# sunkafei/coffeedb

Hardware: AMD Instinct MI355X
Metric: sa_build_GiB_per_s (higher is better)
Workload: dtype u64

## Files before the change

coffeedb_amd/csrc/capi.hip:

```cpp
#include <dirent.h>

#include <algorithm>
#include <chrono>
#include <condition_variable>
#include <cstdlib>
#include <cstring>
#include <thread>

#include "../../include/coffeedb_gpu.h"
#include "index_impl.h"

using namespace cdb;

namespace {

static_assert((int)Status::Invalid == CDB_E_INVALID && (int)Status::Device == CDB_E_DEVICE && (int)Status::Internal == CDB_E_INTERNAL,
              "errors.h: Status restates the CDB_E_* codes");

void set_error(Index& ix, const std::string& msg) {
    std::lock_guard<std::mutex> g(ix.err_mu);
    ix.err = msg;
}

template <typename F>
// ... 1501 lines not shown
        out->nrows = r.nrows;
        out->nhits = r.nhits;
        out->d_row_ptr = ix.q_rowptr.as<uint64_t>();
        out->d_ids = ix.q_ids.as<int64_t>();
        out->d_counts = ix.q_counts.as<int64_t>();
        if (hits) {
            hits->d_hit_ptr = ix.q_hitptr.as<uint64_t>();
            hits->d_offsets = ix.q_hitoff.as<uint64_t>();
        }
        ix.qstats.query_ms = wall_ms() - t0;
        ix.qstats.nhits = r.nhits;
        ix.qstats.nrows = r.nrows;
    });
}
}

int cdb_query_batch_device(cdb_index* h, const void* d_blob, const uint64_t* d_offsets, uint64_t npat,
                           uint64_t blob_bytes, cdb_device_result* out) {
    (void)blob_bytes;
    return query_batch_device_impl(h, d_blob, d_offsets, npat, out, nullptr);
}

int cdb_query_batch_offsets_device(cdb_index* h, const void* d_blob, const uint64_t* d_offsets, uint64_t npat,
                                   uint64_t blob_bytes, cdb_device_result* out, cdb_device_hits* hits) {
    (void)blob_bytes;
    if (!hits) return CDB_E_INVALID;
    return query_batch_device_impl(h, d_blob, d_offsets, npat, out, hits);
}

uint64_t cdb_size(const cdb_index* h) { return h ? h->ix.size : 0; }
uint64_t cdb_bits(const cdb_index* h) { return h ? h->ix.bits : 0; }
uint64_t cdb_mask(const cdb_index* h) { return h ? h->ix.mask : 0; }
int cdb_sa_width(const cdb_index* h) { return h ? h->ix.width : 0; }

int cdb_sa_copy(cdb_index* h, void* host_out, uint64_t capacity_bytes) {
    if (!h || !host_out) return CDB_E_INVALID;
    return guarded(h, [&] {
        Index& ix = h->ix;
        std::lock_guard<std::mutex> g(ix.mu);
        DeviceScope dscope(ix);
        const uint64_t need = ix.size * (uint64_t)ix.width;
        if (capacity_bytes < need) throw Error("cdb_sa_copy: buffer too small");
        if (need && ix.sa_packed) {
            DevBuf chunk;
            const uint64_t per = std::min<uint64_t>(ix.size, 32ull << 20);
            chunk.alloc(per * 8);
            for (uint64_t first = 0; first < ix.size; first += per) {
                const uint64_t cnt = std::min<uint64_t>(per, ix.size - first);
                sa_expand(ix, first, cnt, chunk.as<uint64_t>());
                CDB_HIP(hipMemcpyAsync(static_cast<char*>(host_out) + first * 8, chunk.p, cnt * 8, hipMemcpyDeviceToHost, ix.stream));
                CDB_HIP(hipStreamSynchronize(ix.stream));
            }
        } else if (need) {
            CDB_HIP(hipMemcpyAsync(host_out, ix.d_sa.p, need, hipMemcpyDeviceToHost, ix.stream));
            CDB_HIP(hipStreamSynchronize(ix.stream));
        }
    });
}

int cdb_set_option(cdb_index* h, const char* name, int64_t value) {
    if (!h || !name) return CDB_E_INVALID;
    Index& ix = h->ix;
    for (const char* o : {"fast_search", "key_directory", "single_query", "search_lanes", "keep_keys", "reference_compat"})
        if (!std::strcmp(name, o)) {
            std::lock_guard<std::mutex> g(ix.mu);
            query_resident_stop(ix);
        }
    if (!std::strcmp(name, "profile")) ix.prof.enabled = value != 0;
    else if (!std::strcmp(name, "reference_compat")) ix.reference_compat = value != 0;
    else if (!std::strcmp(name, "force_doubling")) ix.force_doubling = value != 0;
    else if (!std::strcmp(name, "initial_passes")) ix.initial_passes = (int)value;
    else if (!std::strcmp(name, "sort_variant")) ix.sort_variant = (int)value;
    else if (!std::strcmp(name, "keyhist3")) ix.keyhist3 = value != 0;
    else if (!std::strcmp(name, "key_symbols")) ix.key_symbols = (int)value;
    else if (!std::strcmp(name, "msd_first")) ix.msd_first = value != 0;
    else if (!std::strcmp(name, "msd_pair")) ix.msd_pair = value != 0;
    else if (!std::strcmp(name, "overlap_paircount")) ix.overlap_paircount = value != 0;
    else if (!std::strcmp(name, "key_directory")) { ix.key_directory = value != 0; ix.h_keydir.clear(); ix.keydir_tried = false; }
    else if (!std::strcmp(name, "fuse_records")) ix.fuse_records = value != 0;
    else if (!std::strcmp(name, "sweep_records")) ix.sweep_records = value != 0;
    else if (!std::strcmp(name, "partial_symbol")) ix.partial_symbol = value != 0;
    else if (!std::strcmp(name, "group_sort")) ix.group_sort = value != 0;
    else if (!std::strcmp(name, "list_rounds")) ix.list_rounds = value != 0;
    else if (!std::strcmp(name, "fuse_pairclass")) ix.fuse_pairclass = value != 0;
    else if (!std::strcmp(name, "group_sort_cap")) ix.group_sort_cap = (int)std::max<int64_t>(1, std::min<int64_t>(value, 1 << 20));
    else if (!std::strcmp(name, "vl_keys")) ix.vl_keys = value < 0 ? 0 : (value > 56 ? 56 : (int)value);
    else if (!std::strcmp(name, "pack_sa")) ix.pack_sa = value != 0;
    else if (!std::strcmp(name, "key_cost_model")) ix.key_cost_model = value != 0;
    else if (!std::strcmp(name, "gen_prebased")) ix.gen_prebased = value != 0;
    else if (!std::strcmp(name, "pack_entries")) ix.pack_entries = value != 0;
    else if (!std::strcmp(name, "segmented_sort")) ix.segmented_sort = value != 0;
    else if (!std::strcmp(name, "fold_root")) ix.fold_root = value != 0;
    else if (!std::strcmp(name, "fold_depth1")) ix.fold_depth1 = value != 0;
    else if (!std::strcmp(name, "flags_in_last_pass")) ix.flags_in_last_pass = value != 0;
    else if (!std::strcmp(name, "search_lanes")) ix.search_lanes = (value == 1 || value == 8) ? (int)value : 0;
    else if (!std::strcmp(name, "digit_bits")) ix.digit_bits = (int)value;
    else if (!std::strcmp(name, "fuse_keygen")) ix.fuse_keygen = value != 0;
    else if (!std::strcmp(name, "force_big_path")) ix.force_big_path = value != 0;
    else if (!std::strcmp(name, "debug_fail_build")) ix.debug_fail_build = value != 0;
    else if (!std::strcmp(name, "debug_append_path")) ix.debug_append_path = value == 1 || value == 2 ? (int)value : 0;
    else if (!std::strcmp(name, "debug_no_segcap")) ix.debug_no_segcap = value != 0;
    else if (!std::strcmp(name, "debug_starve_group")) ix.debug_starve_group = (int)value;
    else if (!std::strcmp(name, "self_check")) ix.self_check = value < 0 ? 0 : value > 3 ? 3 : (int)value;
    else if (!std::strcmp(name, "premap_generation")) ix.premap_generation = value != 0;
    else if (!std::strcmp(name, "proof_cancel")) {
        if (value) proof_stop(ix);
    }
    else if (!std::strcmp(name, "debug_damage_after_build")) ix.debug_damage_after_build = value < 0 ? 0 : (uint64_t)value;
    else if (!std::strcmp(name, "debug_fail_self_check")) ix.debug_fail_self_check = value != 0;
    else if (!std::strcmp(name, "plain_tile_order")) ix.rws.plain_order = value != 0;
    else if (!std::strcmp(name, "key_coding")) ix.key_coding = (int)value;
    else if (!std::strcmp(name, "narrow_keys")) ix.narrow_keys = value != 0;
    else if (!std::strcmp(name, "single_query")) ix.use_single_query = value != 0;
    else if (!std::strcmp(name, "resident_query")) {
        std::lock_guard<std::mutex> g(ix.mu);
        if (value != 1) query_resident_stop(ix);
        ix.resident_mode = value <= 0 ? 0 : value == 1 ? 1 : 2;
        ix.resident_query = ix.resident_mode == 1;
        ix.single_streak = 0;
    }
    else if (!std::strcmp(name, "bucket_group_limit")) ix.bucket_group_limit = (uint64_t)value;
    else if (!std::strcmp(name, "query_hit_budget"))
        ix.query_hit_budget = value > 0 ? std::min<uint64_t>((uint64_t)value, 1ull << 31) : 1;
    else if (!std::strcmp(name, "coalesce_queries")) ix.coalesce_queries = value != 0;
    else if (!std::strcmp(name, "fast_search")) ix.use_fast_search = value != 0;
    else if (!std::strcmp(name, "wave_rows")) ix.use_wave_rows = value != 0;
    else if (!std::strcmp(name, "keep_keys")) ix.keep_keys = value != 0;
    else {
        set_error(ix, std::string("unknown option: ") + name);
        return CDB_E_INVALID;
    }
    return CDB_OK;
}

int cdb_get_stat(const cdb_index* h, const char* name, double* value) {
    if (!h || !name || !value) return CDB_E_INVALID;
    const BuildStats& b = h->ix.bstats;
    const QueryStats& q = h->ix.qstats;
    struct { const char* n; double v; } tab[] = {
        {"build_ms", b.build_ms}, {"alloc_ms", b.alloc_ms}, {"free_ms", b.free_ms}, {"rounds", (double)b.rounds}, {"ext_rounds", (double)b.ext_rounds},
        {"dbl_rounds", (double)b.dbl_rounds}, {"unresolved_after_initial", (double)b.unresolved_initial},
        {"unresolved_max", (double)b.unresolved_max}, {"sort_passes", (double)b.sort_passes},
        {"sort_passes_skipped", (double)b.sort_passes_skipped}, {"isa_built", (double)b.isa_built}, {"fused_keygen", (double)b.fused_keygen}, {"dense_keys", (double)b.dense_keys}, {"key_layout", (double)b.key_layout}, {"bucketed", (double)b.bucketed}, {"bucket_groups", (double)b.bucket_groups}, {"segmented", (double)b.segmented}, {"fused_records", (double)b.fused_records}, {"sweep_records", (double)b.sweep_records}, {"vl_key_bits", (double)b.vl_key_bits}, {"partial_levels", (double)b.partial_levels}, {"list_rounds", (double)b.list_rounds}, {"pairclass_fused", (double)b.pairclass_fused}, {"group_sorts", (double)b.group_sorts}, {"group_sort_fallbacks", (double)b.group_sort_fallbacks}, {"vl_avg_len", b.vl_avg_len}, {"vl_rate", b.vl_rate}, {"vl_est_unresolved", b.vl_est_unresolved}, {"fixed_est_unresolved", b.fixed_est_unresolved}, {"gen_prebased", (double)b.gen_prebased}, {"root_folded", (double)b.root_folded}, {"flags_in_last_pass", (double)b.flags_in_last_pass}, {"msd_first", (double)b.msd_first}, {"bucket_low_digits", (double)b.bucket_low_digits}, {"key_directory_cells", h->ix.h_keydir.empty() ? 0.0 : (double)(h->ix.h_keydir.size() - 1)}, {"group_fallbacks", (double)h->ix.group_fallbacks}, {"dense_key_retries", (double)h->ix.dense_key_retries}, {"self_check_fallbacks", (double)h->ix.self_check_fallbacks}, {"sa_packed", h->ix.sa_packed ? 1.0 : 0.0}, {"sa_bytes_per_entry", h->ix.sa_packed ? 5.0 : (double)h->ix.width}, {"self_check_pairs", (double)h->ix.self_check_pairs}, {"self_check_ms", h->ix.self_check_ms}, {"self_check_coverage", h->ix.size > 1 ? (double)h->ix.self_check_pairs / (double)(h->ix.size - 1) : 0.0},
        {"order_proved", (h->ix.proof.state.load() == 2 || h->ix.proof.state.load() == 3 || (h->ix.self_check == 2 && h->ix.width != 0)) ? 1.0 : 0.0},
        {"proof_state", (double)h->ix.proof.state.load()}, {"proof_ms", h->ix.proof.ms}, {"proof_repair_ms", h->ix.proof.repair_ms},
        {"proof_pairs", (double)h->ix.proof.pairs}, {"proof_bad_pairs", (double)h->ix.proof.found[0]}, {"proof_invalid_entries", (double)h->ix.proof.found[1]}, {"proof_skipped_pairs", (double)h->ix.proof.skipped}, {"proof_mixed_pairs", (double)h->ix.proof.mixed},
        {"proof_runs", (double)h->ix.proof.runs}, {"pool_big_mallocs", (double)DevPool::get().big_mallocs()}, {"premap_ms", h->ix.proof.premap_ms}, {"premap_bytes", (double)h->ix.proof.premap_bytes},
        {"key_symbols", (double)b.key_symbols}, {"symbol_bits", (double)b.symbol_bits},
        {"alphabet", (double)b.alphabet}, {"digit_bits", (double)b.digit_bits}, {"final_depth", (double)b.final_depth}, {"compat_rotations", (double)b.compat_rotations},
        {"compat_depth", (double)b.compat_depth},
        {"host_upload_ms", h->ix.host_upload_ms}, {"host_free_ms", h->ix.host_free_ms},
        {"resident_answers", (double)h->ix.res_answers}, {"launched_answers", (double)h->ix.launched_answers}, {"resident_mode", (double)h->ix.resident_mode},
        {"cluster_table_bytes", h->ix.clu.valid ? (double)(h->ix.clu.bytes() + h->ix.idt.bytes()) : 0.0}, {"cluster_classes", (double)h->ix.clu.nclasses},
        {"cluster_prepare_ms", h->ix.clu.prepare_ms}, {"cluster_ms", h->ix.clu.last_ms}, {"cluster_resorted", h->ix.clu.resorted ? 1.0 : 0.0},
        {"removes", (double)h->ix.rm.calls}, {"remove_compactions", (double)h->ix.rm.compactions}, {"remove_rebuilds", (double)h->ix.rm.rebuilds},
        {"remove_docs", (double)h->ix.rm.docs}, {"remove_bytes", (double)h->ix.rm.bytes}, {"remove_ms", h->ix.rm.last_ms},
        {"appends", (double)h->ix.ap.calls}, {"append_merges", (double)h->ix.ap.merges}, {"append_rebuilds", (double)h->ix.ap.rebuilds},
        {"append_docs", (double)h->ix.ap.docs}, {"append_bytes", (double)h->ix.ap.bytes}, {"append_ms", h->ix.ap.last_ms},
        {"append_keys_kept", (double)h->ix.ap.with_keys},
        {"render_ms", h->ix.rnd.last_ms}, {"render_page_bytes", (double)h->ix.rnd.page_bytes}, {"render_spans", (double)h->ix.rnd.spans},
        {"query_ms", q.query_ms}, {"query_upload_ms", q.upload_ms}, {"query_device_ms", q.device_ms}, {"query_download_ms", q.download_ms}, {"query_hits", (double)q.nhits}, {"query_rows", (double)q.nrows},
        {"query_batches", (double)q.batches}, {"query_spec_batches", (double)q.spec_batches}, {"query_spec_spills", (double)q.spec_spills},
        {"query_wave_batches", (double)q.wave_batches}, {"query_sort_batches", (double)q.sort_batches}, {"query_sort_chunks", (double)q.sort_chunks},
        {"query_empty_batches", (double)q.empty_batches},
    };
    for (auto& e : tab)
        if (!std::strcmp(e.n, name)) {
            *value = e.v;
            return CDB_OK;
        }
    return CDB_E_INVALID;
}

int cdb_profile_get(cdb_index* h, const char* kernel, double* total_ms, uint64_t* launches, uint64_t* bytes) {
    if (!h || !kernel) return CDB_E_INVALID;
    std::lock_guard<std::mutex> g(h->ix.mu);
    auto it = h->ix.prof.recs.find(kernel);
    if (it == h->ix.prof.recs.end()) return CDB_E_INVALID;
    if (total_ms) *total_ms = it->second.ms;
    if (launches) *launches = it->second.launches;
    if (bytes) *bytes = it->second.bytes;
    return CDB_OK;
}

int cdb_profile_dump(cdb_index* h, char* buf, size_t cap) {
    if (!h || !buf || cap == 0) return CDB_E_INVALID;
    std::lock_guard<std::mutex> g(h->ix.mu);
    std::string s;
    for (auto& kv : h->ix.prof.recs) {
        char line[256];
        std::snprintf(line, sizeof(line), "%s %.6f %llu %llu\n", kv.first.c_str(), kv.second.ms,
                      (unsigned long long)kv.second.launches, (unsigned long long)kv.second.bytes);
        s += line;
    }
    std::strncpy(buf, s.c_str(), cap - 1);
    buf[cap - 1] = 0;
    return CDB_OK;
}

int cdb_debug_verify(cdb_index* h, uint64_t out[5]) {
    if (!h || !out) return CDB_E_INVALID;
    return guarded(h, [&] {
        Index& ix = h->ix;
        std::lock_guard<std::mutex> g(ix.mu);
        DeviceScope dscope(ix);
        if (ix.width == 0) throw Error("index has not been built");
        verify_suffix_array(ix, out);
    });
}

int cdb_debug_self_check(cdb_index* h, int full, uint64_t out[2]) {
    if (!h || !out) return CDB_E_INVALID;
    return guarded(h, [&] {
        Index& ix = h->ix;
        std::lock_guard<std::mutex> g(ix.mu);
        DeviceScope dscope(ix);
        if (ix.width == 0) throw Error("index has not been built");
        spot_check_suffix_array(ix, full ? 0u : (uint32_t)std::min<uint64_t>(1u << 15, ix.size > 1 ? ix.size - 1 : 1), out);
    });
}

int cdb_proof_wait(cdb_index* h, double timeout_ms) {
    if (!h) return CDB_E_INVALID;
    const double t0 = wall_ms();
    for (;;) {
        const int st = h->ix.proof.state.load();
// ... 94 lines not shown
```

coffeedb_amd/csrc/index_impl.h:

```cpp
#pragma once
#include <atomic>
#include <condition_variable>
#include <functional>
#include <mutex>
#include <thread>
#include <string>
#include <vector>

#include "../../include/coffeedb_gpu.h"
#include "common.h"
#include "radix_sort.h"

namespace cdb {

constexpr int TEXT_PAD = 128;

struct BuildStats {
    double build_ms = 0, alloc_ms = 0, free_ms = 0;
    int rounds = 0;
    int ext_rounds = 0;
    int dbl_rounds = 0;
    uint64_t unresolved_initial = 0;
    uint64_t unresolved_max = 0;
    int sort_passes = 0;
    int sort_passes_skipped = 0;
    int isa_built = 0;
    int fused_keygen = 0;
    int key_layout = 0;
    int dense_keys = 0;
    int bucketed = 0;
    int bucket_low_digits = 0;
    int bucket_groups = 0;
    int root_folded = 0;
    int flags_in_last_pass = 0;
    int msd_first = 0;
    int gen_prebased = 0;
    int fused_records = 0;
    int sweep_records = 0;
    int pairclass_fused = 0;
    int list_rounds = 0;
    int group_sorts = 0, group_sort_fallbacks = 0;
    int partial_levels = 0;
    int vl_key_bits = 0;
    double vl_avg_len = 0, vl_rate = 0, vl_est_unresolved = 0, fixed_est_unresolved = 0;
    int segmented = 0;
    uint64_t gather_items = 0;
    int key_symbols = 0, symbol_bits = 0, alphabet = 0, digit_bits = 8;
    uint64_t final_depth = 0;
    uint64_t compat_rotations = 0, compat_depth = 0;
};

struct QueryStats {
    double query_ms = 0;
    double upload_ms = 0, device_ms = 0, download_ms = 0;
    uint64_t nhits = 0, nrows = 0;
    uint64_t batches = 0;
    uint64_t spec_batches = 0, spec_spills = 0;
    uint64_t wave_batches = 0;
    uint64_t sort_batches = 0, sort_chunks = 0;
    uint64_t empty_batches = 0;
};

struct KeptKeys {
    uint64_t* k64 = nullptr;
    uint32_t* k32 = nullptr;
    uint8_t* low = nullptr;
    int low_bits = 0, low_bytes = 0;
    __host__ __device__ __forceinline__ bool present() const { return k64 != nullptr || k32 != nullptr; }
    __device__ __forceinline__ uint64_t low_at(uint64_t i) const {
        return low_bytes == 2 ? (uint64_t)reinterpret_cast<const uint16_t*>(low)[i] : (uint64_t)low[i];
    }
    __device__ __forceinline__ uint64_t at(uint64_t i) const {
        if (k64) return k64[i];
        const uint64_t h = k32[i];
        if (!low_bits) return h;
        return (h << low_bits) | low_at(i);
    }
    __device__ __forceinline__ int cmp_range(uint64_t i, uint64_t klo, uint64_t khi) const {
        uint64_t key;
        if (k64) {
            key = k64[i];
        } else {
            const uint64_t h = k32[i];
            if (low) {
                const uint64_t a = klo >> low_bits, b = khi >> low_bits;
                if (h < a) return -1;
                if (h > b) return 1;
                if (h > a && h < b) return 0;
                key = (h << low_bits) | low_at(i);
            } else {
                key = h;
            }
        }
        return key < klo ? -1 : (key > khi ? 1 : 0);
    }
    __device__ __forceinline__ void put(uint64_t i, uint64_t key) const {
        if (k64) k64[i] = key;
        if (k32) k32[i] = (uint32_t)(key >> low_bits);
        if (low) {
            const uint64_t l = key & ((1ull << low_bits) - 1ull);
            if (low_bytes == 2) reinterpret_cast<uint16_t*>(low)[i] = (uint16_t)l;
            else low[i] = (uint8_t)l;
        }
    }
    __device__ __forceinline__ void copy(const KeptKeys& src, uint64_t from, uint64_t to) const {
        if (k64) k64[to] = src.k64[from];
        if (k32) k32[to] = src.k32[from];
        if (low) {
            if (low_bytes == 2) reinterpret_cast<uint16_t*>(low)[to] = reinterpret_cast<const uint16_t*>(src.low)[from];
            else low[to] = src.low[from];
        }
    }
    uint64_t bytes_per_slot() const { return (k64 ? 8 : 0) + (k32 ? 4 : 0) + (low ? low_bytes : 0); }
};
struct SingleKeys {
    KeptKeys keys;
    int nsym = 0;
    bool decisive = false;
    uint64_t klo = 0, khi = 0;
    bool ranged = false;
    uint64_t lo0 = 0, hi0 = 0;
};

struct Sa40 {
// ... 54 lines not shown
    bool overlap_paircount = true;
    bool res_running = false;
    uint32_t res_seq = 0;
    SingleKeys res_keys;
    bool use_fast_search = true;

    std::vector<int64_t> ids;
    std::vector<uint64_t> doc_start{0};
    std::string host_text;
    bool host_tables_valid = true;
    bool host_text_valid = true;

    uint64_t bits = 1, mask = 1, size = 0;
    int off_bits = 1;
    int width = 0;
    uint64_t ndocs = 0;

    DevBuf d_text_owned;
    const uint8_t* d_text = nullptr;
    bool text_padded = false;
    DevBuf d_doc_start;
    DevBuf d_ids;
    DevBuf d_sa;
    DevBuf d_sa_hi;
    bool sa_packed = false;
    bool gen_prebased = true;
    TileBaseWorkspace tbw;
    bool key_cost_model = true;
    bool pack_sa = true;
    void release_sa() {
        d_sa.release();
        d_sa_hi.release();
        sa_packed = false;
        clu.drop();
        idt.drop();
    }
    template <typename T> typename SaOf<T>::ptr sa_view() const;
    bool sa_sorted = false;
    DevBuf d_keys;
    DevBuf d_symmap_q;
    uint16_t h_symmap_q[256] = {};
    DevBuf d_keys32, d_keylow;
    int key_low_bits = 0;
    int key_low_bytes = 0;
    int key_nsym = 0;
    uint32_t key_base = 0;
    void drop_keys() {
        d_keys.release();
        d_keys32.release();
        d_keylow.release();
        key_nsym = 0;
        key_low_bits = 0;
        key_low_bytes = 0;
        h_keydir.clear();
        h_keydir.shrink_to_fit();
        keydir_tried = false;
    }
    std::vector<uint32_t> h_keydir;
    int keydir_shift = 0, keydir_bits = 0;
    bool keydir_tried = false;
    bool key_directory = true;
    DevBuf d_pivots;
    int pivot_levels = 0;

    RadixWorkspace rws;
    MsdWorkspace msd_ws;
    DevBuf scan_partials;
    uint64_t q_spec_cap = 0;
    DevBuf q_spec;
    DevBuf q_pat, q_offs, q_left, q_right, q_hoff, q_keys0, q_keys1, q_flags, q_rowptr, q_ids, q_counts, q_hitptr, q_hitoff;

    bool reference_compat = true;
    bool force_doubling = false;
    int initial_passes = 0;
    int key_symbols = 0;
    int sort_variant = 0;
    int search_lanes = 0;
    bool flags_in_last_pass = true;
    bool fold_depth1 = true;
    bool fold_root = true;
    bool segmented_sort = true;
    bool fuse_records = true;
    bool fuse_pairclass = true;
    bool list_rounds = true;
    int group_sort_cap = 4096;
    bool group_sort = true;
    bool partial_symbol = true;
    int vl_keys = 2;
    bool vl_off_once = false;
    bool sweep_records = true;
    bool pack_entries = true;
    bool msd_first = true;
    bool msd_pair = true;
    bool keyhist3 = true;
    int dense_key_retries = 0;
    int group_fallbacks = 0;
    uint64_t bucket_group_limit = 0;
    uint64_t self_check_pairs = 0;
    double self_check_ms = 0;
    int self_check = 3;
    int self_check_fallbacks = 0;
    bool debug_fail_self_check = false;
    struct Proof {
        std::thread th;
        std::atomic<int> state{0};
        std::atomic<bool> cancel{false};
        hipStream_t stream = nullptr;
        void* d_out = nullptr;
        double ms = 0, repair_ms = 0;
        uint64_t pairs = 0;
        uint64_t found[2] = {0, 0};
        uint64_t skipped = 0;
        uint64_t mixed = 0;
        uint64_t runs = 0;
        bool of_loaded_file = false;
        std::atomic<bool> busy{false};
        bool want_proof = false;
        double premap_ms = 0;
        uint64_t premap_bytes = 0;
    } proof;
    bool premap_generation = false;
    bool proof_in_repair = false;
    uint64_t debug_damage_after_build = 0;
    bool debug_no_segcap = false;
    int debug_starve_group = 0;
    bool debug_fail_build = false;
    bool force_big_path = false;
    bool fuse_keygen = true;
    int digit_bits = 0;
    bool narrow_keys = true;
    int key_coding = 0;
    uint64_t query_hit_budget = 1ull << 31;

    struct ClusterTables {
        bool valid = false;
        uint64_t nclasses = 0;
        bool resorted = false;
        DevBuf class_of_doc;
        DevBuf class_rep;
        double prepare_ms = 0, last_ms = 0;
        uint64_t bytes() const { return class_of_doc.bytes + class_rep.bytes; }
        void drop() {
            valid = false;
            nclasses = 0;
            class_of_doc.release();
            class_rep.release();
        }
    } clu;
    struct IdTable {
        bool valid = false;
        bool ids_ascend = true;
        DevBuf id_sorted, id_doc;
        uint64_t bytes() const { return id_sorted.bytes + id_doc.bytes; }
        void drop() {
            valid = false;
            ids_ascend = true;
            id_sorted.release();
            id_doc.release();
        }
    } idt;
    struct RenderStats {
        double last_ms = 0;
        uint64_t page_bytes = 0, spans = 0;
    } rnd;

    struct RemoveStats {
// ... 227 lines not shown
```

coffeedb_amd/csrc/radix_sort.h:

```cpp
#pragma once
#include <cstdlib>

#include "common.h"

namespace cdb {

constexpr int RS_MAX_PASSES = 16;

constexpr uint64_t RS_VAL_MASK = (1ull << 54) - 1;
constexpr uint32_t RS_SPIN_LIMIT_GROUPED = 1u << 18;
constexpr uint32_t RS_SPIN_LIMIT_PLAIN = 1u << 22;
constexpr int RS_GROUP = 8;

struct NoVal {};

template <typename K>
__global__ __launch_bounds__(256) void rs_hist_kernel(const K* __restrict__ keys, uint64_t n, int begin_bit,
                                                      int npass, int dbits, uint32_t last_mask,
                                                      unsigned long long* __restrict__ ghist) {
    __shared__ uint32_t sh[RS_MAX_PASSES * 256];
    for (int i = threadIdx.x; i < npass * 256; i += 256) sh[i] = 0;
    __syncthreads();
    const uint64_t stride = (uint64_t)gridDim.x * 256;
    for (uint64_t i = (uint64_t)blockIdx.x * 256 + threadIdx.x; i < n; i += stride) {
// ... 108 lines not shown
    int rec_low_bits = 0;
    uint32_t part_m = 1, part_r = 0, part_s = 0;
    bool msd_pair = false;
    uint32_t pair_span = 0, pair_r = 0, pair_s = 0;
    const uint64_t* tile_doc = nullptr;
    const unsigned long long* tile_base = nullptr;
    uint8_t* vout_hi = nullptr;
};
struct TextGenPair : TextGen {};
struct TextGenRec : TextGen {};
constexpr int RS_GEN_LOOK = 64;
#ifndef RS_GEN_ABL
#define RS_GEN_ABL 0
#endif
#ifndef RS_SEG_ABL
#define RS_SEG_ABL 0
#endif



struct RsDiv24 { uint32_t mul, sh; };
inline RsDiv24 rs_div24_make(uint32_t d) {
    uint32_t L = 0;
    while ((1ull << L) < d) ++L;
    const uint64_t m = ((1ull << (24 + L)) + d - 1) / d;
    return RsDiv24{(uint32_t)(m << 7), L + 7};
}
__device__ __forceinline__ uint32_t rs_div24(uint32_t x, uint32_t mul, uint32_t sh) { return __umulhi(x << 8, mul) >> sh; }

template <typename G>
inline bool rs_pair_setup(G& gen, uint32_t base, uint32_t span) {
    const uint64_t b2 = (uint64_t)base * base;
    if (base < 2 || base > 255 || span == 0 || span >= (1u << 24) || b2 >= (1u << 24)) return false;
    if ((uint64_t)span * b2 >= (1u << 24)) return false;
    if ((uint64_t)span * b2 * b2 > (1ull << 32)) return false;
    for (uint32_t sh = 0; sh < 32; ++sh) {
        const uint64_t r = ((1ull << sh) + span - 1) / span;
        if (r >= (1u << 24) || (b2 - 1) * r >= (1ull << 32)) break;
        bool ok = true;
        for (uint64_t a = 0; a < b2 && ok; ++a) ok = ((a * r) >> sh) == a / span;
        if (ok) {
            gen.pair_span = span;
            gen.pair_r = (uint32_t)r;
            gen.pair_s = sh;
            return true;
        }
    }
    return false;
}

struct NoSeg {};
struct SegInfo {
    unsigned long long begin, end;
    uint32_t tile_begin, top;
    unsigned long long rot_a, rot_b;
};
__device__ __forceinline__ unsigned long long rs_seg_rotated(const SegInfo& si, unsigned long long slot) {
    if (si.rot_b == 0) return slot;
    const unsigned long long r = slot - si.begin, len = si.end - si.begin;
    if (r < si.rot_a) return slot;
    return r < si.rot_b ? slot + (len - si.rot_b) : slot - (si.rot_b - si.rot_a);
}
struct SegArgs {
    const uint32_t* tile_seg = nullptr;
    const SegInfo* segs = nullptr;
    uint32_t tiles = 0;
    uint32_t start_stride = 0;
};
struct SegEdge {
    unsigned long long first, last;
    unsigned long long pos;
    uint32_t cnt, pad;
};
struct SegFinalArgs : SegArgs {
    uint64_t* eout = nullptr;
    uint32_t* elo = nullptr;
    uint8_t* ehi = nullptr;
    uint8_t* flags = nullptr;
    SegEdge* edges = nullptr;
    int hi_shift = 0;
    int low_bits = 0;
    uint32_t kbase = 2;
    unsigned long long kmagic = 0;
};

struct SegFinalKeepArgs : SegArgs {
    uint8_t* flags = nullptr;
    SegEdge* edges = nullptr;
    int low_bits = 0;
    uint32_t kbase = 2;
    unsigned long long kmagic = 0;
    unsigned long long* tile_sums = nullptr;
    uint32_t sums_tile = 1;
    unsigned long long msd_m = 0;
};

struct SegFinalKeepMsdArgs : SegFinalKeepArgs {};

__device__ __forceinline__ uint64_t rs_pack_key(const uint32_t* __restrict__ s_words, uint32_t li, int nsym, uint32_t base,
                                                uint32_t rem) {
    const uint32_t wi = li >> 2, sel = li & 3u;
    const uint32_t b2 = base * base, b3 = b2 * base;
    const uint32_t pw[5] = {1u, base, b2, b3, b3 * base};
    uint64_t kk = 0;
    uint32_t lo = s_words[wi];
#pragma unroll
    for (int w = 0; w < 4; ++w) {
        const int q = 4 * w;
        if (q >= nsym) break;
        const int r = nsym - q < 4 ? nsym - q : 4;
        const uint32_t hi = s_words[wi + w + 1];
        uint32_t x = __builtin_amdgcn_alignbyte(hi, lo, sel);
        lo = hi;
        if (rem < (uint32_t)(q + 4)) x = rem <= (uint32_t)q ? 0u : (x & ((1u << (8u * (rem - (uint32_t)q))) - 1u));
        uint32_t v = x & 0xFFu;
        if (r > 1) v = v * base + ((x >> 8) & 0xFFu);
        if (r > 2) v = v * base + ((x >> 16) & 0xFFu);
        if (r > 3) v = v * base + (x >> 24);
        kk = (r == 4 && pw[4] == 0u) ? ((kk << 32) | v) : kk * pw[r] + v;
    }
    return kk;
}

__device__ __forceinline__ uint64_t rs_doc_upper(const uint64_t* __restrict__ doc_start, uint64_t lo, uint64_t hi,
                                                 uint64_t p) {
    while (lo < hi) {
        const uint64_t mid = lo + (hi - lo + 1) / 2;
        if (doc_start[mid] <= p) lo = mid; else hi = mid - 1;
    }
    return lo;
}

static __global__ __launch_bounds__(256) void rs_tiledoc_kernel(const uint64_t* __restrict__ doc_start, uint64_t ndocs,
                                                                uint64_t n, uint64_t tile_elems, uint64_t tiles,
                                                                uint64_t* __restrict__ tile_doc) {
    const uint64_t t = (uint64_t)blockIdx.x * 256 + threadIdx.x;
    if (t > tiles) return;
    const uint64_t p = t * tile_elems < n ? t * tile_elems : n - 1;
    tile_doc[t] = rs_doc_upper(doc_start, 0, ndocs - 1, p);
}

template <typename K, typename V, typename Cfg, typename Gen = NoGen, typename W = NoVal, typename Seg = NoSeg>
__global__ __launch_bounds__(Cfg::NT, Cfg::MINW) void rs_onesweep_kernel(
    const K* __restrict__ kin, K* __restrict__ kout, const V* __restrict__ vin, V* __restrict__ vout, uint64_t n,
    int shift, uint32_t dmask, const unsigned long long* __restrict__ digit_start, uint64_t* __restrict__ status,
    uint32_t* __restrict__ ticket, uint32_t epoch, uint32_t* __restrict__ err, Gen gen = Gen(),
    const W* __restrict__ win = nullptr, W* __restrict__ wout = nullptr, int aux_shift = -1, Seg seg = Seg()) {
    constexpr bool GEN = !std::is_same<Gen, NoGen>::value;
    constexpr bool SEG = !std::is_same<Seg, NoSeg>::value;
    constexpr bool FINAL = std::is_same<Seg, SegFinalArgs>::value;
    constexpr bool KEEPM = std::is_same<Seg, SegFinalKeepMsdArgs>::value;
    constexpr bool KEEP = std::is_same<Seg, SegFinalKeepArgs>::value || KEEPM;
    constexpr bool FLAGS = FINAL || KEEP;
    static_assert(!SEG || (!GEN && !Cfg::DMA), "segmented passes: materialised records");
    static_assert(!FLAGS || Cfg::REUSE || KEEPM, "flag-writing passes: shared staging (the MSD-first last pass also runs with keys and values staged at once)");
    constexpr bool HAS_V = !std::is_same<V, NoVal>::value;
    constexpr bool HAS_W = !std::is_same<W, NoVal>::value;
    using WS = typename std::conditional<HAS_W, W, uint8_t>::type;
    static_assert(!HAS_W || KEEPM || (Cfg::REUSE && HAS_V && !Cfg::DMA), "the auxiliary byte needs the shared-staging configuration");
    constexpr int IPT = Cfg::IPT;
    constexpr bool REUSE = Cfg::REUSE && HAS_V;
    constexpr bool EARLYV = (Cfg::EARLYV || REUSE) && HAS_V;
    constexpr int NT = Cfg::NT;
    constexpr int NW = NT / 64;
    constexpr bool NTM = Cfg::NONTEMP;
    constexpr int TILE = NT * IPT;
// ... 611 lines not shown
            if (real) {
                const uint64_t lmask = (1ull << seg.low_bits) - 1ull;
                const uint32_t a = tstart, b = tstart + (uint32_t)real - 1u;
                if constexpr (KEEPM) {
                    e.first = ktop + (uint64_t)s_keys[a];
                    e.last = ktop + (uint64_t)s_keys[b];
                } else {
                    e.first = ((uint64_t)s_keys[a] << seg.low_bits) | ((uint64_t)s_aux[HAS_W ? a : 0] & lmask);
                    e.last = ((uint64_t)s_keys[b] << seg.low_bits) | ((uint64_t)s_aux[HAS_W ? b : 0] & lmask);
                }
            }
            seg.edges[tile * 256 + d] = e;
        }
    }

    if constexpr (!REUSE) {
#pragma unroll
        for (int j = 0; j < IPT; ++j) {
            const uint32_t i = j * NT + tid;
            if (i < valid) {
                const K k = s_keys[i];
                const uint32_t dd = (uint32_t)(k >> shift) & dmask;
                const uint64_t dst = s_gbase[dd] + i;
                if constexpr (KEEPM) {
                    bool head = true, tail = true;
                    if (i > 0) head = s_keys[i - 1] != k;
                    if (i + 1 < valid) tail = s_keys[i + 1] != k;
                    const uint64_t kf = ktop + (uint64_t)k;
                    uint32_t f = head ? 1u : 0u;
                    if (!(head && tail)) {
                        const bool exhausted = seg.kmagic ? (kf - __umul64hi(kf, seg.kmagic) * seg.kbase) == 0
                                                          : (kf & (uint64_t)(seg.kbase - 1u)) == 0;
                        if (!exhausted) f |= 2u;
                    }
                    seg.flags[dst] = (uint8_t)f;
                    if ((f & 2u) && seg.tile_sums) {
                        atomicAdd(seg.tile_sums + 2 * (dst / seg.sums_tile), 1ull);
                        if (f & 1u) atomicAdd(seg.tile_sums + 2 * (dst / seg.sums_tile) + 1, 1ull);
                    }
                    rs_store<NTM>(kout + dst, (K)(kf >> 8));
                    if constexpr (HAS_W) rs_store<NTM>(wout + dst, (W)(kf & 0xFFu));
                    rs_store<NTM>(vout + dst, (V)s_vals[i]);
                    continue;
                }
                if (!GEN || kout) rs_store<NTM>(kout + dst, k);
                if constexpr (HAS_V) rs_store<NTM>(vout + dst, (V)s_vals[i]);
            }
        }
    } else {
        uint8_t dig[IPT];
#pragma unroll
        for (int j = 0; j < IPT; ++j) {
            const uint32_t i = j * NT + tid;
            dig[j] = 0;
            if (i < valid) {
                const K k = s_keys[i];
                uint32_t dd;
                if constexpr (KEEPM) dd = (uint32_t)(k >> shift) & dmask;
                else dd = digit_of(k, s_aux[HAS_W ? i : 0]);
                if constexpr (recs) dd = (uint32_t)s_gen[i];
                dig[j] = (uint8_t)dd;
                if constexpr (FLAGS) {
                    const uint32_t lmask = seg.low_bits >= 32 ? 0xFFFFFFFFu : (1u << seg.low_bits) - 1u;
                    uint32_t ac = 0;
                    if constexpr (!KEEPM) ac = (uint32_t)s_aux[HAS_W ? i : 0] & lmask;
                    bool head = true, tail = true;
                    bool cmp = true;
                    if constexpr (FINAL) cmp = !(RS_SEG_ABL & 4);
                    if constexpr (KEEPM) {
                        if (i > 0) head = s_keys[i - 1] != k;
                        if (i + 1 < valid) tail = s_keys[i + 1] != k;
                    } else if (cmp) {
                        if (i > 0) head = s_keys[i - 1] != k || ((uint32_t)s_aux[HAS_W ? i - 1 : 0] & lmask) != ac;
                        if (i + 1 < valid) tail = s_keys[i + 1] != k || ((uint32_t)s_aux[HAS_W ? i + 1 : 0] & lmask) != ac;
                    }
                    uint32_t f = head ? 1u : 0u;
                    if (!(head && tail)) {
                        const uint64_t kc = KEEPM ? ktop + (uint64_t)k : (((uint64_t)k << seg.low_bits) | (uint64_t)ac);
                        const bool exhausted = seg.kmagic ? (kc - __umul64hi(kc, seg.kmagic) * seg.kbase) == 0
                                                          : (kc & (uint64_t)(seg.kbase - 1u)) == 0;
                        if (!exhausted) f |= 2u;
                    }
                    if constexpr (FINAL) {
                        if (!(RS_SEG_ABL & 1)) seg.flags[rs_seg_rotated(si, s_gbase[dd] + i)] = (uint8_t)f;
                        continue;
                    } else {
                        const uint64_t slot = s_gbase[dd] + i;
                        seg.flags[slot] = (uint8_t)f;
                        if ((f & 2u) && seg.tile_sums) {
                            atomicAdd(seg.tile_sums + 2 * (slot / seg.sums_tile), 1ull);
                            if (f & 1u) atomicAdd(seg.tile_sums + 2 * (slot / seg.sums_tile) + 1, 1ull);
                        }
                    }
                }
                if constexpr (KEEPM) {
                    const uint64_t kf = ktop + (uint64_t)k;
                    rs_store<NTM>(kout + s_gbase[dd] + i, (K)(kf >> 8));
                    if constexpr (HAS_W) rs_store<NTM>(wout + s_gbase[dd] + i, (W)(kf & 0xFFu));
                    continue;
                }
                if (!GEN || kout) rs_store<NTM>(kout + s_gbase[dd] + i, k);
                if constexpr (HAS_W && !W32G) {
                    if (!GEN || wout) rs_store<NTM>(wout + s_gbase[dd] + i, (W)s_aux[i]);
                }
            }
        }
        __syncthreads();
        if constexpr (W32G) {
#pragma unroll
            for (int j = 0; j < IPT; ++j) s_vals[rank[j]] = (VS)aux[j];
            __syncthreads();
#pragma unroll
            for (int j = 0; j < IPT; ++j) {
                const uint32_t i = j * NT + tid;
                if (i < valid) rs_store<NTM>(wout + s_gbase[dig[j]] + i, (W)s_vals[i]);
            }
            __syncthreads();
        }
#pragma unroll
        for (int j = 0; j < IPT; ++j) s_vals[rank[j]] = val[j];
        __syncthreads();
#pragma unroll
        for (int j = 0; j < IPT; ++j) {
            const uint32_t i = j * NT + tid;
            if constexpr (FINAL) {
                if (i < valid && !(RS_SEG_ABL & 2)) {
                    const unsigned long long slot = rs_seg_rotated(si, s_gbase[dig[j]] + i);
                    const uint32_t hi32 = (uint32_t)s_aux[HAS_W ? i : 0] >> seg.hi_shift;
                    if (seg.elo) {
                        seg.elo[slot] = (uint32_t)s_vals[i];
                        seg.ehi[slot] = (uint8_t)hi32;
                    } else {
                        seg.eout[slot] = ((uint64_t)hi32 << 32) | (uint64_t)s_vals[i];
                    }
                }
            } else {
                if constexpr (GEN && sizeof(VS) == 8) {
                    if (gen.vout_hi) {
                        if (i < valid) {
                            const uint64_t dst = s_gbase[dig[j]] + i;
                            const uint64_t e = (uint64_t)s_vals[i];
                            reinterpret_cast<uint32_t*>(vout)[dst] = (uint32_t)e;
                            gen.vout_hi[dst] = (uint8_t)(e >> 32);
                        }
                        continue;
                    }
                }
                if (i < valid) rs_store<NTM>(vout + s_gbase[dig[j]] + i, (V)s_vals[i]);
            }
        }
    }
}

static __global__ __launch_bounds__(256) void rs_seg_edge_fix_kernel(const SegEdge* __restrict__ edges, const uint32_t* __restrict__ tile_seg,
                                                                     const SegInfo* __restrict__ segs, uint32_t tiles,
                                                                     uint8_t* __restrict__ flags, uint32_t kbase, unsigned long long kmagic,
                                                                     unsigned long long* __restrict__ tile_sums = nullptr,
                                                                     uint32_t sums_tile = 1, const uint32_t* __restrict__ err = nullptr) {
    const uint32_t t = blockIdx.x, d = threadIdx.x;
    if (t >= tiles) return;
    if (err && *err) return;
    const SegEdge e = edges[(size_t)t * 256 + d];
    if (!e.cnt) return;
    const SegInfo si = segs[tile_seg ? tile_seg[t] : 0u];
    const uint32_t t0 = si.tile_begin;
    if (t == t0) return;
    uint32_t lo = t0, hi = t;
    if (edges[(size_t)(t - 1) * 256 + d].pos < e.pos) {
        lo = t - 1;
    } else {
        if (edges[(size_t)t0 * 256 + d].pos >= e.pos) return;
        hi = t - 1;
        while (hi - lo > 1) {
            const uint32_t mid = lo + (hi - lo) / 2;
            if (edges[(size_t)mid * 256 + d].pos < e.pos) lo = mid; else hi = mid;
        }
    }
    const SegEdge pe = edges[(size_t)lo * 256 + d];
    if (pe.last != e.first) return;
    const bool exhausted = kmagic ? (e.first - __umul64hi(e.first, kmagic) * kbase) == 0 : (e.first & (uint64_t)(kbase - 1u)) == 0;
    auto change = [&](unsigned long long slot, uint32_t clear, uint32_t set) {
        const uintptr_t a = reinterpret_cast<uintptr_t>(flags + slot);
        unsigned int* w = reinterpret_cast<unsigned int*>(a & ~(uintptr_t)3);
        const uint32_t sh = 8u * (uint32_t)(a & 3u);
        uint32_t before, after;
        if (clear) {
            before = (atomicAnd(w, ~(clear << sh)) >> sh) & 0xFFu;
            after = before & ~clear;
        } else {
            before = (atomicOr(w, set << sh) >> sh) & 0xFFu;
            after = before | set;
        }
        if (tile_sums && before != after) {
            const long long da = (long long)((after >> 1) & 1u) - (long long)((before >> 1) & 1u);
            const long long db = (long long)((after >> 1) & after & 1u) - (long long)((before >> 1) & before & 1u);
            unsigned long long* ts = tile_sums + 2 * (slot / sums_tile);
            if (da) atomicAdd(ts, (unsigned long long)da);
            if (db) atomicAdd(ts + 1, (unsigned long long)db);
        }
    };
    const unsigned long long sb = rs_seg_rotated(si, e.pos), sa_ = rs_seg_rotated(si, e.pos - 1);
    change(sb, 1u, 0u);
    if (!exhausted) {
        change(sb, 0u, 2u);
        change(sa_, 0u, 2u);
    }
}

static __global__ __launch_bounds__(256) void rs_lane_order_probe_kernel(uint32_t* __restrict__ bad) {
    __shared__ uint32_t cnt[4][256];
    __shared__ uint32_t ref[4][256];
// ... 861 lines not shown
```

coffeedb_amd/csrc/records_sweep.h:

```cpp
#pragma once
#include "radix_sort.h"

namespace cdb {

#ifndef RS_SWEEP_ABL
#define RS_SWEEP_ABL 0
#endif
#ifndef RS_SWEEP_UNALIGNED
#define RS_SWEEP_UNALIGNED 0
#endif
__device__ __forceinline__ int rs_uniform(int x) {
    int y = __builtin_amdgcn_readfirstlane(x);
    asm volatile("" : "+s"(y));
    return y;
}
__device__ __forceinline__ uint32_t rs_wave_incl_scan(uint32_t x) {
    uint32_t v = x;
    v += (uint32_t)__builtin_amdgcn_update_dpp(0, (int)x, 0x111, 0xf, 0xf, false);
    v += (uint32_t)__builtin_amdgcn_update_dpp(0, (int)x, 0x112, 0xf, 0xf, false);
    v += (uint32_t)__builtin_amdgcn_update_dpp(0, (int)x, 0x113, 0xf, 0xf, false);
    v += (uint32_t)__builtin_amdgcn_update_dpp(0, (int)v, 0x114, 0xf, 0xe, false);
    v += (uint32_t)__builtin_amdgcn_update_dpp(0, (int)v, 0x118, 0xf, 0xc, false);
    v += (uint32_t)__builtin_amdgcn_update_dpp(0, (int)v, 0x142, 0xa, 0xf, false);
    v += (uint32_t)__builtin_amdgcn_update_dpp(0, (int)v, 0x143, 0xc, 0xf, false);
    return v;
}

constexpr int RS_SWEEP_TILE = RS_GEN8_TILE;
constexpr uint32_t RS_SWEEP_DOCS = 768;

template <typename W>
__global__ __launch_bounds__(512, 8) void rs_sweep_records_kernel(TextGen gen, const uint16_t* __restrict__ codeslot, uint64_t n, uint32_t tiles,
                                                                  uint32_t g0, uint32_t g1, uint64_t gstart, uint32_t* __restrict__ kout,
                                                                  uint32_t* __restrict__ vout, W* __restrict__ wout) {
    constexpr int NT = 512, IPT = 16, TILE = RS_SWEEP_TILE, NW = NT / 64;
    static_assert(NT * IPT == TILE, "tile shape");
    constexpr int abl = RS_SWEEP_ABL;
    constexpr uint32_t TEXTB = ((TILE + RS_GEN_LOOK + 15) / 16) * 16;
    constexpr uint32_t NBLK = TILE / 32, DOCS = 184;
    __shared__ __attribute__((aligned(16))) uint8_t s_text[TEXTB];
    __shared__ uint16_t s_cs[256];
    __shared__ __attribute__((aligned(16))) uint32_t s_doc[4 * DOCS];
    __shared__ uint8_t s_slotc[256];
    __shared__ uint32_t s_whist[NW][256];
    __shared__ __attribute__((aligned(8))) uint32_t s_blk[2 * (NBLK + 1)];
    __shared__ uint64_t s_gbase[256];
    __shared__ uint32_t s_wsum[8];
    __shared__ uint32_t s_flag;
    __shared__ __attribute__((aligned(16))) uint16_t s_idx[TILE];
    uint8_t* const s_dig = reinterpret_cast<uint8_t*>(s_idx);

    const int tid = threadIdx.x, lane = tid & 63, wave = tid >> 6;
    const uint32_t x = blockIdx.x & 7u, slot = blockIdx.x >> 3;
    const uint64_t tile = (uint64_t)((slot / RS_GROUP) * 8u + x) * RS_GROUP + slot % RS_GROUP;
    if (tile >= (uint64_t)tiles) return;
    const uint64_t base = tile * TILE;
    const uint32_t valid = (uint32_t)((n - base) < (uint64_t)TILE ? (n - base) : (uint64_t)TILE);

    const uint64_t ga = base + (uint64_t)tid * 16, gb = base + (uint64_t)TILE + (uint64_t)tid * 16;
    const bool has_b = (uint32_t)tid * 16 < TEXTB - (uint32_t)TILE;
    const bool oka = gen.padded ? (ga < n + RS_GEN_LOOK) : (ga + 16 <= n);
    const bool okb = has_b && (gen.padded ? (gb < n + RS_GEN_LOOK) : (gb + 16 <= n));
    uint4 ta = make_uint4(0, 0, 0, 0), tb = make_uint4(0, 0, 0, 0);
    if (oka) ta = *reinterpret_cast<const uint4*>(gen.text + ga);
    if (okb) tb = *reinterpret_cast<const uint4*>(gen.text + gb);
    uint64_t my_base = 0;
    if ((uint32_t)tid >= g0 && (uint32_t)tid < g1) my_base = (uint64_t)gen.tile_base[tile * 256 + (uint64_t)tid];
    if (tid < 256) {
        const uint32_t e = codeslot[tid];
        s_cs[tid] = (uint16_t)(((e >> 8) >= g0 && (e >> 8) < g1) ? e : (e | 0xFF00u));
        s_slotc[tid] = gen.slotmap[tid];
    }
    const uint64_t dlo = gen.tile_doc[tile], dhi = gen.tile_doc[tile + 1];
    for (int i = tid; i < NW * 256; i += NT) (&s_whist[0][0])[i] = 0;
    if ((uint32_t)tid <= NBLK) s_blk[2 * tid] = 0;
    if (tid == 0) s_flag = 0;
    const uint32_t ndl = (uint32_t)(dhi - dlo);
    const bool docs_in_lds = dhi - dlo + 2 <= (uint64_t)DOCS;
    uint64_t dreg0 = 0;
    if (docs_in_lds && (uint32_t)tid < ndl + 2) dreg0 = gen.doc_start[dlo + tid];
    __syncthreads();
    if (docs_in_lds && (uint32_t)tid < ndl + 2) {
        const uint32_t d = (uint32_t)tid;
        const int64_t diff = (int64_t)(dreg0 - base);
// ... 124 lines not shown
        const uint32_t l1 = li + 1u, wi = l1 >> 2, sel = l1 & 3u;
        const uint32_t w0 = s_words[wi], w1 = s_words[wi + 1], w2 = s_words[wi + 2];
        uint32_t x0 = __builtin_amdgcn_alignbyte(w1, w0, sel);
        uint32_t x1 = __builtin_amdgcn_alignbyte(w2, w1, sel);
        uint32_t x2 = 0;
        if (nsx > 8) x2 = __builtin_amdgcn_alignbyte(s_words[wi + 3], w2, sel);
        if (__builtin_expect(__builtin_amdgcn_readfirstlane((int)(__builtin_amdgcn_ballot_w64(rem1 < (uint32_t)nsx) != 0)) != 0, 0)) {
            if (rem1 < (uint32_t)nsx) {
                x0 = rem1 >= 4u ? x0 : (rem1 == 0u ? 0u : (x0 & ((1u << (8u * rem1)) - 1u)));
                x1 = rem1 >= 8u ? x1 : (rem1 <= 4u ? 0u : (x1 & ((1u << (8u * (rem1 - 4u))) - 1u)));
                x2 = rem1 >= 12u ? x2 : (rem1 <= 8u ? 0u : (x2 & ((1u << (8u * (rem1 - 8u))) - 1u)));
            }
        }
        uint64_t acc = 0;
#pragma unroll
        for (int q = 0; q < 5; ++q) {
            if (2 * q < ns1) {
                const uint32_t xw = q < 2 ? x0 : (q < 4 ? x1 : x2);
                uint32_t pv, mult;
                if (2 * q + 1 < ns1) {
                    pv = __builtin_amdgcn_udot4(xw, (q & 1) ? whi : wlo, 0u, false);
                    mult = B2;
                } else {
                    pv = (q & 1) ? ((xw >> 16) & 0xFFu) : (xw & 0xFFu);
                    mult = B;
                }
                if (q == 0) acc = pv;
                else if (q == 1) acc = (uint64_t)(uint32_t)acc * mult + pv;
                else acc = acc * (uint64_t)mult + pv;
            }
        }
        if (part_on) {
            const uint32_t xq = ns1 < 4 ? x0 : (ns1 < 8 ? x1 : x2);
            const uint32_t cq = (xq >> (8 * (ns1 & 3))) & 0xFFu;
            acc = acc * (uint64_t)gen.part_m + (uint64_t)((cq * gen.part_r) >> gen.part_s);
        }
        const uint64_t dst = s_gbase[sl] + (uint64_t)p;
        if (abl & 8) {
            if (acc == 0x123456789ull && e64 == 77) kout[dst] = 1;
            return;
        }
        kout[dst] = (uint32_t)(acc >> gen.rec_low_bits);
        vout[dst] = (uint32_t)e64;
        wout[dst] = (W)((acc & lmask) | ((e64 >> 32) << gen.rec_low_bits));
    };
    if (docs_in_lds && s_flag == 0 && valid == (uint32_t)TILE && !(abl & 4)) {
        const int bits = gen.bits;
        auto rec = [&](uint32_t p) {
            const uint32_t li = s_idx[p];
            const uint2 bk = *reinterpret_cast<const uint2*>(&s_blk[2 * (li >> 5)]);
            const uint32_t doff = bk.y + 16u * (uint32_t)__builtin_popcount(bk.x & ~(0xFFFFFFFEu << (li & 31u)));
            const uint4 dc = *reinterpret_cast<const uint4*>(reinterpret_cast<const uint8_t*>(s_doc) + doff);
            emit(p, li, (((uint64_t)dc.y << 32) | dc.x) + ((uint64_t)li << bits), (uint32_t)((int32_t)dc.z - (int32_t)li - 1));
        };
        if (kept == (uint32_t)TILE) {
            for (uint32_t p = tid; p < (uint32_t)TILE; p += 2 * NT) {
                rec(p);
                rec(p + NT);
            }
        } else {
            for (uint32_t p = tid; p < kept; p += NT) rec(p);
        }
    } else {
        for (uint32_t p = tid; p < kept; p += NT) {
            const uint32_t li = s_idx[p];
            const uint64_t pos = base + li;
            uint64_t dd = dlo, ds = 0, de = 1ull << 40;
            if (!(abl & 4)) {
                dd = rs_doc_upper(gen.doc_start, dlo, dhi, pos);
                ds = gen.doc_start[dd];
                de = gen.doc_start[dd + 1];
            }
            const uint64_t left = de - pos - 1ull;
            emit(p, li, ((pos - ds) << gen.bits) + dd, left < 64ull ? (uint32_t)left : 64u);
        }
    }
}

struct VlTables {
    const uint16_t* sym = nullptr;
    const uint16_t* dec = nullptr;
    int key_bits = 0;
    int end_len = 0;
};
constexpr uint32_t RS_VL_BITW = ((RS_GEN8_TILE + RS_GEN_LOOK) * 7 + 31) / 32 + 4;

template <typename W>
__global__ __launch_bounds__(512, 6) void rs_sweep_records_vl_kernel(TextGen gen, const uint16_t* __restrict__ codeslot, VlTables vl, uint64_t n,
                                                                     uint32_t tiles, uint32_t g0, uint32_t g1, uint64_t gstart,
                                                                     uint32_t* __restrict__ kout, uint32_t* __restrict__ vout, W* __restrict__ wout) {
    constexpr int NT = 512, IPT = 16, TILE = RS_SWEEP_TILE, NW = NT / 64;
    constexpr uint32_t LOOK = RS_GEN_LOOK, NBLK = TILE / 32, DOCS = 256, SL = 128;
    static_assert(LOOK == 64, "four staging threads cover the look-ahead");
    __shared__ uint32_t s_bits[RS_VL_BITW];
    __shared__ __attribute__((aligned(16))) uint16_t s_boff[TILE + LOOK + 8];
    __shared__ __attribute__((aligned(16))) uint16_t s_idx[TILE];
    __shared__ uint32_t s_whist[NW][SL];
    __shared__ uint16_t s_cs[256];
    __shared__ uint16_t s_vl[SL];
    __shared__ uint16_t s_dec[128];
    __shared__ __attribute__((aligned(16))) uint32_t s_doc[4 * DOCS + 4];
    __shared__ __attribute__((aligned(8))) uint32_t s_blk[2 * (NBLK + 1)];
    __shared__ uint64_t s_gbase[SL];
    __shared__ uint32_t s_wsum[16];
    __shared__ uint32_t s_flag;
    uint8_t* const s_dig = reinterpret_cast<uint8_t*>(s_idx);

    const int tid = threadIdx.x, lane = tid & 63, wave = tid >> 6;
    const uint32_t x = blockIdx.x & 7u, slot = blockIdx.x >> 3;
    const uint64_t tile = (uint64_t)((slot / RS_GROUP) * 8u + x) * RS_GROUP + slot % RS_GROUP;
    if (tile >= (uint64_t)tiles) return;
    const uint64_t base = tile * TILE;
    const uint32_t valid = (uint32_t)((n - base) < (uint64_t)TILE ? (n - base) : (uint64_t)TILE);

    const uint64_t ga = base + (uint64_t)tid * 16, gb = base + (uint64_t)TILE + (uint64_t)tid * 16;
    const bool has_b = (uint32_t)tid * 16 < LOOK;
    const bool oka = gen.padded ? (ga < n + LOOK) : (ga + 16 <= n);
    const bool okb = has_b && (gen.padded ? (gb < n + LOOK) : (gb + 16 <= n));
    uint4 ta = make_uint4(0, 0, 0, 0), tb = make_uint4(0, 0, 0, 0);
    if (oka) ta = *reinterpret_cast<const uint4*>(gen.text + ga);
    if (okb) tb = *reinterpret_cast<const uint4*>(gen.text + gb);
    uint64_t my_base = 0;
    if ((uint32_t)tid >= g0 && (uint32_t)tid < g1) my_base = (uint64_t)gen.tile_base[tile * 256 + (uint64_t)tid];
    if (tid < 256) {
        const uint32_t e = codeslot[tid];
        s_cs[tid] = (uint16_t)(((e >> 8) >= g0 && (e >> 8) < g1) ? e : (e | 0xFF00u));
    }
    if (tid < (int)SL) {
        s_vl[tid] = vl.sym[tid];
        s_dec[tid] = vl.dec[tid];
    }
    const uint64_t dlo = gen.tile_doc[tile], dhi = gen.tile_doc[tile + 1];
    for (int i = tid; i < NW * (int)SL; i += NT) (&s_whist[0][0])[i] = 0;
    for (uint32_t i = tid; i < RS_VL_BITW; i += NT) s_bits[i] = 0;
    if ((uint32_t)tid <= NBLK) s_blk[2 * tid] = 0;
    if (tid == 0) s_flag = 0;
    const uint32_t ndl = (uint32_t)(dhi - dlo);
    const bool docs_in_lds = dhi - dlo + 2 <= (uint64_t)DOCS;
    uint64_t dreg0 = 0;
    if (docs_in_lds && (uint32_t)tid < ndl + 2) dreg0 = gen.doc_start[dlo + tid];
    __syncthreads();
    if (docs_in_lds && (uint32_t)tid < ndl + 2) {
        const uint32_t d = (uint32_t)tid;
        const int64_t diff = (int64_t)(dreg0 - base);
        const int32_t rel = diff < -(1ll << 30) ? -(1 << 30) : (diff > (1ll << 30) ? (1 << 30) : (int32_t)diff);
        const uint64_t eb = ((base - dreg0) << gen.bits) + dlo + d;
        s_doc[4 * d] = (uint32_t)eb;
        s_doc[4 * d + 1] = (uint32_t)(eb >> 32);
        if (d >= 1) s_doc[4 * d - 2] = (uint32_t)rel;
        if (d >= 1 && rel <= (int32_t)TILE) {
            const uint32_t bit = 1u << ((uint32_t)rel & 31u);
            if (atomicOr(&s_blk[2 * ((uint32_t)rel >> 5)], bit) & bit) s_flag = 1;
        }
    }
    auto fetch = [&](uint64_t g, bool ok, uint4 w, uint32_t* c) {
        c[0] = w.x; c[1] = w.y; c[2] = w.z; c[3] = w.w;
        if (!ok) {
#pragma unroll
            for (int q = 0; q < 4; ++q) {
                c[q] = 0;
#pragma unroll
                for (int b = 0; b < 4; ++b) c[q] |= (uint32_t)((g + 4 * q + b < n) ? gen.text[g + 4 * q + b] : (uint8_t)0) << (8 * b);
            }
        }
    };
    auto pack4 = [&](const uint32_t* v, uint32_t& word, uint32_t& wlen, uint32_t& lens4) {
// ... 60 lines not shown
                o += (lens[k >> 3] >> (4 * (k & 7))) & 0xFu;
            }
            *reinterpret_cast<uint4*>(&s_boff[pos0]) = make_uint4(packed[0], packed[1], packed[2], packed[3]);
            *reinterpret_cast<uint4*>(&s_boff[pos0 + 8]) = make_uint4(packed[4], packed[5], packed[6], packed[7]);
            uint32_t bo = at;
#pragma unroll
            for (int h = 0; h < 2; ++h) {
                const uint32_t wi = bo >> 5, sh = bo & 31u;
                const uint32_t xh = (uint32_t)(piece[h] >> 32), xl = (uint32_t)piece[h];
                atomicOr(&s_bits[wi], __builtin_amdgcn_alignbit(0u, xh, sh));
                atomicOr(&s_bits[wi + 1], __builtin_amdgcn_alignbit(xh, xl, sh));
                atomicOr(&s_bits[wi + 2], __builtin_amdgcn_alignbit(xl, 0u, sh));
                bo += plen[h];
            }
            return o;
        };
        (void)emit_bits(wpre + inclA - totA, pieceA, plenA, lensA, (uint32_t)tid * 16);
        if (has_b) {
            const uint32_t end = emit_bits(all + inclB - totB, pieceB, plenB, lensB, (uint32_t)TILE + (uint32_t)tid * 16);
            if ((uint32_t)tid * 16 + 16 == LOOK) s_boff[TILE + LOOK] = (uint16_t)end;
        }
    }
    __syncthreads();
    constexpr int WCHUNK = IPT * 64;
    const uint32_t wbase = wave * WCHUNK + lane;
    uint32_t info[IPT];
    {
        uint32_t sl[IPT];
#pragma unroll
        for (int j = 0; j < IPT; ++j) sl[j] = s_dig[wbase + j * 64];
#pragma unroll
        for (int j = 0; j < IPT; ++j) {
            uint32_t inf = 0xFFu << 16;
            if (sl[j] != 0xFFu) inf = atomicAdd(&s_whist[wave][sl[j]], 1u) | (sl[j] << 16);
            info[j] = inf;
        }
    }
    __syncthreads();
    uint32_t wc[NW], cnt = 0, incl = 0;
    if (tid < (int)SL) {
#pragma unroll
        for (int w = 0; w < NW; ++w) {
            wc[w] = s_whist[w][tid];
            cnt += wc[w];
        }
        incl = cnt;
    } else if (tid >= 256) {
        incl = cnt = (uint32_t)__builtin_popcount(s_blk[2 * (tid - 256)]);
    }
    incl = rs_wave_incl_scan(incl);
    if (lane == 63) s_wsum[8 + wave] = incl;
    __syncthreads();
    const uint32_t kept = s_wsum[8] + s_wsum[9];
    {
        uint32_t wpre = 0;
        if (tid < (int)SL) {
            if (wave == 1) wpre = s_wsum[8];
            const uint32_t excl = wpre + incl - cnt;
            uint32_t run = excl;
#pragma unroll
            for (int w = 0; w < NW; ++w) {
                s_whist[w][tid] = run;
                run += wc[w];
            }
            s_gbase[tid] = my_base - gstart - (uint64_t)excl;
        } else if (tid >= 256) {
#pragma unroll
            for (int w = 4; w < NW; ++w)
                if (w < wave) wpre += s_wsum[8 + w];
            const uint32_t excl = wpre + incl - cnt;
            s_blk[2 * (tid - 256) + 1] = excl * 16u;
            if (tid == 511) s_blk[2 * NBLK + 1] = (excl + cnt) * 16u;
        }
    }
    __syncthreads();
#pragma unroll
    for (int k = 0; k < IPT; ++k) {
        const uint32_t sl = info[k] >> 16;
        if (sl != 0xFFu) s_idx[s_whist[wave][sl] + (info[k] & 0xFFFFu)] = (uint16_t)(wbase + k * 64);
    }
    __syncthreads();

    const int KB1 = vl.key_bits - 1;
    const uint64_t lmask = (1ull << gen.rec_low_bits) - 1ull;
    auto emit = [&](uint32_t p, uint32_t li, uint64_t e64, uint32_t endbit) {
        const uint32_t o0 = s_boff[li];
        const uint32_t wi = o0 >> 5, sh = o0 & 31u;
        const uint32_t w0 = s_bits[wi], w1 = s_bits[wi + 1], w2 = s_bits[wi + 2];
        const uint32_t hi = __builtin_amdgcn_alignbit(w0, w1, 32u - sh), lo = __builtin_amdgcn_alignbit(w1, w2, 32u - sh);
        const uint64_t top = sh ? (((uint64_t)hi << 32) | lo) : (((uint64_t)w0 << 32) | w1);
        const uint32_t dv = s_dec[(uint32_t)(top >> 57)];
        const uint32_t sl = dv & 0xFFu, len = dv >> 8;
        const uint32_t avail = endbit - (o0 + len);
        const uint32_t take = avail < (uint32_t)KB1 ? avail : (uint32_t)KB1;
        uint64_t kb = (top << len) >> (64 - KB1);
        kb &= ~0ull << ((uint32_t)KB1 - take);
        const uint64_t key = (kb << 1) | (uint64_t)(avail + (uint32_t)vl.end_len > (uint32_t)KB1 ? 1u : 0u);
        const uint64_t dst = s_gbase[sl] + (uint64_t)p;
        kout[dst] = (uint32_t)(key >> gen.rec_low_bits);
        vout[dst] = (uint32_t)e64;
        wout[dst] = (W)((key & lmask) | ((e64 >> 32) << gen.rec_low_bits));
    };
    if (docs_in_lds && s_flag == 0 && valid == (uint32_t)TILE) {
        const int bits = gen.bits;
        for (uint32_t p = tid; p < kept; p += NT) {
            const uint32_t li = s_idx[p];
            const uint2 bk = *reinterpret_cast<const uint2*>(&s_blk[2 * (li >> 5)]);
            const uint32_t doff = bk.y + 16u * (uint32_t)__builtin_popcount(bk.x & ~(0xFFFFFFFEu << (li & 31u)));
            const uint4 dc = *reinterpret_cast<const uint4*>(reinterpret_cast<const uint8_t*>(s_doc) + doff);
            const int32_t rn = (int32_t)dc.z;
            const uint32_t relend = rn < (int32_t)(TILE + LOOK) ? (uint32_t)rn : (uint32_t)(TILE + LOOK);
            emit(p, li, (((uint64_t)dc.y << 32) | dc.x) + ((uint64_t)li << bits), (uint32_t)s_boff[relend]);
        }
    } else {
        for (uint32_t p = tid; p < kept; p += NT) {
            const uint32_t li = s_idx[p];
            const uint64_t pos = base + li;
            const uint64_t dd = rs_doc_upper(gen.doc_start, dlo, dhi, pos);
            const uint64_t ds = gen.doc_start[dd], de = gen.doc_start[dd + 1];
            const uint64_t rel = de - base;
            const uint32_t relend = rel < (uint64_t)(TILE + LOOK) ? (uint32_t)rel : (uint32_t)(TILE + LOOK);
            emit(p, li, ((pos - ds) << gen.bits) + dd, (uint32_t)s_boff[relend]);
        }
    }
}

__global__ __launch_bounds__(512, 8) void rs_sweep_msd_kernel(TextGen gen, uint64_t n, uint32_t tiles, uint32_t* __restrict__ kout,
                                                              uint32_t* __restrict__ vout) {
    constexpr int NT = 512, IPT = 16, TILE = RS_SWEEP_TILE, NW = NT / 64;
    constexpr uint32_t TEXTB = ((TILE + RS_GEN_LOOK + 15) / 16) * 16;
    constexpr uint32_t DOCS = 384;
    constexpr uint32_t NBLK = TILE / 32;
    __shared__ __attribute__((aligned(16))) uint8_t s_text[TEXTB];
    __shared__ uint8_t s_code[256];
    __shared__ __attribute__((aligned(8))) uint32_t s_doc[2 * DOCS + 2];
    __shared__ uint32_t s_whist[NW][256];
    __shared__ __attribute__((aligned(8))) uint32_t s_blk[2 * (NBLK + 1)];
    __shared__ uint32_t s_gbase[256];
    __shared__ uint32_t s_wsum[8];
    __shared__ uint32_t s_flag;
    __shared__ __attribute__((aligned(16))) uint16_t s_idx[TILE];
    uint8_t* const s_dig = reinterpret_cast<uint8_t*>(s_idx);

    const int tid = threadIdx.x, lane = tid & 63, wave = tid >> 6;
    const uint32_t x = blockIdx.x & 7u, slot = blockIdx.x >> 3;
    const uint64_t tile = (uint64_t)((slot / RS_GROUP) * 8u + x) * RS_GROUP + slot % RS_GROUP;
    if (tile >= (uint64_t)tiles) return;
    const uint64_t base = tile * TILE;
    const uint32_t valid = (uint32_t)((n - base) < (uint64_t)TILE ? (n - base) : (uint64_t)TILE);

    const uint64_t ga = base + (uint64_t)tid * 16, gb = base + (uint64_t)TILE + (uint64_t)tid * 16;
    const bool has_b = (uint32_t)tid * 16 < TEXTB - (uint32_t)TILE;
    const bool oka = gen.padded ? (ga < n + RS_GEN_LOOK) : (ga + 16 <= n);
    const bool okb = has_b && (gen.padded ? (gb < n + RS_GEN_LOOK) : (gb + 16 <= n));
    uint4 ta = make_uint4(0, 0, 0, 0), tb = make_uint4(0, 0, 0, 0);
    if (oka) ta = *reinterpret_cast<const uint4*>(gen.text + ga);
    if (okb) tb = *reinterpret_cast<const uint4*>(gen.text + gb);
    uint32_t tnext = 0;
    if (lane == 63 && ga + 16 < n) tnext = (uint32_t)gen.text[ga + 16];
    uint64_t my_base = 0;
    if (tid < 256) {
        my_base = (uint64_t)gen.tile_base[tile * 256 + (uint64_t)tid];
        s_code[tid] = (uint8_t)gen.symmap[tid];
    }
    const uint64_t dlo = gen.tile_doc[tile], dhi = gen.tile_doc[tile + 1];
    for (int i = tid; i < NW * 256; i += NT) (&s_whist[0][0])[i] = 0;
    if ((uint32_t)tid <= NBLK) s_blk[2 * tid] = 0;
    if (tid == 0) s_flag = 0;
    const uint32_t ndl = (uint32_t)(dhi - dlo);
    const bool docs_in_lds = dhi - dlo + 2 <= (uint64_t)DOCS;
    uint64_t dreg0 = 0, dreg1 = 0;
    if (docs_in_lds) {
        if ((uint32_t)tid < ndl + 2) dreg0 = gen.doc_start[dlo + tid];
        if ((uint32_t)tid + NT < ndl + 2) dreg1 = gen.doc_start[dlo + tid + NT];
    }
    __syncthreads();
    if (docs_in_lds) {
        auto put = [&](uint32_t d, uint64_t ds) {
            const int64_t diff = (int64_t)(ds - base);
            const int32_t rel = diff < -(1ll << 30) ? -(1 << 30) : (diff > (1ll << 30) ? (1 << 30) : (int32_t)diff);
            s_doc[2 * d] = (uint32_t)(((base - ds) << gen.bits) + dlo + d);
            if (d >= 1) s_doc[2 * d - 1] = (uint32_t)rel;
            if (d >= 1 && rel <= (int32_t)TILE) {
                const uint32_t bit = 1u << ((uint32_t)rel & 31u);
// ... 155 lines not shown
        vout[dst] = ent;
    };
    if (docs_in_lds && s_flag == 0 && valid == (uint32_t)TILE) {
        constexpr int U = 2;
        const int bits = gen.bits;
#pragma nounroll
        for (uint32_t p0 = tid; p0 < (uint32_t)TILE; p0 += U * NT) {
            uint32_t li[U];
            uint2 bk[U], dc[U];
#pragma unroll
            for (int u = 0; u < U; ++u) li[u] = s_idx[p0 + u * NT];
#pragma unroll
            for (int u = 0; u < U; ++u) bk[u] = *reinterpret_cast<const uint2*>(&s_blk[2 * (li[u] >> 5)]);
#pragma unroll
            for (int u = 0; u < U; ++u) {
                const uint32_t doff = bk[u].y + 8u * (uint32_t)__builtin_popcount(bk[u].x & ~(0xFFFFFFFEu << (li[u] & 31u)));
                dc[u] = *reinterpret_cast<const uint2*>(reinterpret_cast<const uint8_t*>(s_doc) + doff);
            }
#pragma unroll
            for (int u = 0; u < U; ++u) emit(p0 + u * NT, li[u], dc[u].x + (li[u] << bits), dc[u].y - li[u]);
        }
    } else {
        for (uint32_t p = tid; p < valid; p += NT) {
            const uint32_t li = s_idx[p];
            const uint64_t pos = base + li;
            const uint64_t dd = rs_doc_upper(gen.doc_start, dlo, dhi, pos);
            const uint64_t ds = gen.doc_start[dd], de = gen.doc_start[dd + 1];
            const uint64_t left = de - pos;
            emit(p, li, (uint32_t)(((pos - ds) << gen.bits) + dd), left < 64ull ? (uint32_t)left : 64u);
        }
    }
}

inline bool rs_sweep_records_ok(uint32_t base, int nsym) { return base <= 255u && nsym >= 2 && nsym - 1 <= 10; }
template <typename G>
inline bool rs_part_setup(G& gen, uint32_t base, uint32_t m) {
    gen.part_m = 1;
    gen.part_r = gen.part_s = 0;
    if (m < 2 || base < 2 || base > 256) return false;
    for (uint32_t sh = 0; sh < 24; ++sh) {
        const uint64_t r = (((uint64_t)m << sh) + base - 1) / base;
        if (r >= (1u << 24)) break;
        bool ok = true;
        for (uint64_t c = 0; c < base && ok; ++c) ok = ((c * r) >> sh) == c * m / base;
        if (ok) {
            gen.part_m = m;
            gen.part_r = (uint32_t)r;
            gen.part_s = sh;
            return true;
        }
    }
    return false;
}

template <typename W>
void radix_sweep_records(hipStream_t s, Profiler& prof, uint32_t* k, uint32_t* v, W* w, uint64_t n, const TextGen& gen_in, const uint16_t* d_codeslot,
                         uint32_t g0, uint32_t g1,
                         uint64_t gstart, uint64_t gelems, const uint32_t* d_tile_seg, const SegInfo* d_segs, uint32_t nseg, uint32_t seg_tiles,
                         int lead, int npass, unsigned long long* d_hist_out, SortStats* stats) {
    if (!gen_in.tile_base || !gen_in.tile_doc || !d_codeslot || !gen_in.slotmap) throw InternalError("radix_sweep_records: tile bases / documents / slots missing (internal)");
    if (!rs_sweep_records_ok(gen_in.base, gen_in.nsym)) throw InternalError("radix_sweep_records: key shape (internal)");
    const uint32_t tiles8 = (uint32_t)ceil_div(n, (uint64_t)RS_SWEEP_TILE);
    const uint32_t grid = (uint32_t)(ceil_div(tiles8, 8u * RS_GROUP) * 8u * RS_GROUP);
    CDB_HIP(hipMemsetAsync(d_hist_out, 0, (size_t)nseg * 8 * 256 * sizeof(uint64_t), s));
    int t = prof.begin(s);
    hipLaunchKernelGGL((rs_sweep_records_kernel<W>), dim3(grid), dim3(512), 0, s, gen_in, d_codeslot, n, tiles8, g0, g1, gstart, k, v, w);
    prof.end(t, (std::string("rs_sweep_records") + (sizeof(W) == 1 ? "_w8" : (sizeof(W) == 2 ? "_w16" : "_w32")) + "_t8192").c_str(),
             n + gelems * (8 + sizeof(W)), s);
    if (stats) stats->passes_run++;
    t = prof.begin(s);
    hipLaunchKernelGGL((rs_seg_hist_kernel<W>), dim3((unsigned)ceil_div(seg_tiles, (uint32_t)RS_MSD_HIST_TILES)), dim3(1024), 0, s, (const uint32_t*)k,
                       (const W*)w, lead, npass, d_tile_seg, d_segs, seg_tiles, d_hist_out);
    prof.end(t, "rs_seg_hist", gelems * (4 + (lead > 0 ? sizeof(W) : 0)), s);
    CDB_HIP(hipGetLastError());
}

template <typename W>
void radix_sweep_records_vl(hipStream_t s, Profiler& prof, uint32_t* k, uint32_t* v, W* w, uint64_t n, const TextGen& gen_in, const uint16_t* d_codeslot,
                            const VlTables& vl, uint32_t g0, uint32_t g1, uint64_t gstart, uint64_t gelems, const uint32_t* d_tile_seg,
                            const SegInfo* d_segs, uint32_t nseg, uint32_t seg_tiles, int lead, int npass, unsigned long long* d_hist_out,
                            SortStats* stats) {
    if (!gen_in.tile_base || !gen_in.tile_doc || !d_codeslot || !vl.sym || !vl.dec) throw InternalError("radix_sweep_records_vl: tables missing (internal)");
    if (vl.key_bits < 16 || vl.key_bits > 56) throw InternalError("radix_sweep_records_vl: key width (internal)");
    const uint32_t tiles8 = (uint32_t)ceil_div(n, (uint64_t)RS_SWEEP_TILE);
    const uint32_t grid = (uint32_t)(ceil_div(tiles8, 8u * RS_GROUP) * 8u * RS_GROUP);
    CDB_HIP(hipMemsetAsync(d_hist_out, 0, (size_t)nseg * 8 * 256 * sizeof(uint64_t), s));
    int t = prof.begin(s);
    hipLaunchKernelGGL((rs_sweep_records_vl_kernel<W>), dim3(grid), dim3(512), 0, s, gen_in, d_codeslot, vl, n, tiles8, g0, g1, gstart, k, v, w);
    prof.end(t, (std::string("rs_sweep_records_vl") + (sizeof(W) == 1 ? "_w8" : (sizeof(W) == 2 ? "_w16" : "_w32")) + "_t8192").c_str(),
             n + gelems * (8 + sizeof(W)), s);
    if (stats) stats->passes_run++;
    t = prof.begin(s);
    hipLaunchKernelGGL((rs_seg_hist_kernel<W>), dim3((unsigned)ceil_div(seg_tiles, (uint32_t)RS_MSD_HIST_TILES)), dim3(1024), 0, s, (const uint32_t*)k,
                       (const W*)w, lead, npass, d_tile_seg, d_segs, seg_tiles, d_hist_out);
    prof.end(t, "rs_seg_hist", gelems * (4 + (lead > 0 ? sizeof(W) : 0)), s);
    CDB_HIP(hipGetLastError());
}

}
```

coffeedb_amd/csrc/sa_build.hip:

```cpp
#include <algorithm>
#include <chrono>
#include <cmath>
#include <cstdlib>
#include <cstring>

#include "index_impl.h"
#include "records_sweep.h"
#include "vl_code.h"
#include "scan.h"

#ifndef RS_GATHER_ABL
#define RS_GATHER_ABL 0
#endif

namespace cdb {
namespace {

constexpr int KG_TILE = 2048;
constexpr int KG_LOOK = 64;

__global__ __launch_bounds__(256) void sa_bytecount_kernel(const uint8_t* __restrict__ text, uint64_t n,
                                                           unsigned long long* __restrict__ counts) {
    __shared__ uint32_t s[256];
    s[threadIdx.x] = 0;
// ... 908 lines not shown
#pragma unroll
            for (int u = 0; u < U; ++u) {
                live[u] = r0 + 256u * u < it.count;
                e[u] = live[u] ? ent[it.begin + r0 + 256u * u] : 0ull;
            }
#pragma unroll
            for (int u = 0; u < U; ++u) {
                const uint64_t d = live[u] ? (e[u] & mask) : 0ull;
                if (abl & 2) {
                    pos[u] = (e[u] >> bits) + d * 1024;
                    rem[u] = 1u << 20;
                    continue;
                }
                const uint64_t ds = doc_start[d], de = doc_start[d + 1];
                pos[u] = ds + (e[u] >> bits);
                rem[u] = de - pos[u];
            }
#pragma unroll
            for (int u = 0; u < U; ++u) {
                windowed[u] = live[u] && pos[u] + 24 <= n;
                if (abl & 4) {
                    w0[u] = e[u] * 0x9E3779B97F4A7C15ull;
                    w1[u] = w0[u] >> 7;
                    continue;
                }
                w0[u] = windowed[u] ? *reinterpret_cast<const u64_unaligned*>(text + pos[u] + 1) : 0ull;
                w1[u] = windowed[u] && nsym > 9 ? *reinterpret_cast<const u64_unaligned*>(text + pos[u] + 9) : 0ull;
            }
#pragma unroll
            for (int u = 0; u < U; ++u) {
                if (!live[u]) continue;
                uint64_t key = 0;
                if (windowed[u]) {
                    uint64_t w = w0[u];
                    for (int k = 1; k < nsym && k <= 8; ++k) {
                        key = key * kbase + ((uint64_t)k < rem[u] ? (uint64_t)s_map[w & 0xff] : 0ull);
                        w >>= 8;
                    }
                    w = w1[u];
                    for (int k = 9; k < nsym; ++k) {
                        key = key * kbase + ((uint64_t)k < rem[u] ? (uint64_t)s_map[w & 0xff] : 0ull);
                        w >>= 8;
                    }
                } else {
                    for (int k = 1; k < nsym; ++k)
                        key = key * kbase + ((uint64_t)k < rem[u] ? (uint64_t)s_map[text[pos[u] + k]] : 0ull);
                }
                const uint64_t i = it.begin + r0 + 256u * u;
                k32[i - gstart] = (uint32_t)(key >> low_bits);
                low[i - gstart] = (W)((key & ((1ull << low_bits) - 1ull)) | ((e[u] >> 32) << low_bits));
                if (!(abl & 8)) elo[i - gstart] = (uint32_t)e[u];
                if (!(abl & 1))
                    for (int q = 0; q < npass; ++q) atomicAdd(&s_hist[q][(uint32_t)(key >> (8 * q)) & 0xFFu], 1u);
            }
        }
        __syncthreads();
        unsigned long long* h = hist + (size_t)(it.bucket - bucket0) * 8 * 256;
        for (int p = 0; p < npass; ++p)
            if (s_hist[p][threadIdx.x]) atomicAdd(&h[p * 256 + threadIdx.x], (unsigned long long)s_hist[p][threadIdx.x]);
    }
}

template <typename W>
__global__ __launch_bounds__(256) void sa_assemble_entries_kernel(const uint32_t* __restrict__ elo, const W* __restrict__ low,
                                                                  int hi_shift, uint64_t cnt, uint64_t* __restrict__ out) {
    const uint64_t i = (uint64_t)blockIdx.x * 256 + threadIdx.x;
    if (i < cnt) out[i] = ((uint64_t)((uint32_t)low[i] >> hi_shift) << 32) | (uint64_t)elo[i];
}


template <typename SAW, typename I>
struct CompactOut {
    using V = typename SAW::val;
    SAW sa;
    I* U;
    uint64_t* skey;
    V* sval;
    int kbits;
    __device__ __forceinline__ void operator()(uint64_t i, const U2& ex, const U2& in) const {
        if (in.a == ex.a) return;
        const uint64_t j = ex.a;
        U[j] = (I)i;
        skey[j] = (in.b - 1) << kbits;
        sval[j] = sa.load(i);
    }
};

template <typename V, typename I>
struct CompactListOut {
    const I* Uo;
    const V* svo;
    I* U;
    uint64_t* skey;
    V* sval;
    int kbits;
    __device__ __forceinline__ void operator()(uint64_t j, const U2& ex, const U2& in) const {
        if (in.a == ex.a) return;
        const uint64_t jj = ex.a;
        U[jj] = Uo[j];
        skey[jj] = (in.b - 1) << kbits;
        sval[jj] = svo[j];
    }
};

template <typename V, typename R, bool USE_ISA>
__global__ __launch_bounds__(256) void sa_round_keys_kernel(const V* __restrict__ sval, uint64_t m,
                                                            const uint64_t* __restrict__ doc_start,
                                                            const uint8_t* __restrict__ text,
                                                            const uint16_t* __restrict__ symmap,
                                                            const R* __restrict__ rank, int bits, uint64_t mask, uint64_t h,
                                                            int nsym2, int symbits, uint64_t* __restrict__ skey, uint64_t n_text,
                                                            const uint8_t* __restrict__ vl_len = nullptr, uint32_t vl_kb1 = 0,
                                                            uint32_t h_extra = 0, uint8_t* __restrict__ hcov = nullptr) {
    const uint64_t j = (uint64_t)blockIdx.x * 256 + threadIdx.x;
    if (j >= m) return;
    const V v = sval[j];
    const uint64_t d = (uint64_t)v & mask, off = (uint64_t)v >> bits;
    const uint64_t ds = doc_start[d];
    if (!USE_ISA && vl_len) {
        const uint64_t len = doc_start[d + 1] - ds - off;
        const uint8_t* q = text + ds + off;
        const uint64_t pa = (uint64_t)q & ~7ull;
        const uint32_t sh = (uint32_t)((uint64_t)q & 7ull) * 8u;
        const uint64_t tend = (uint64_t)(text + n_text);
        const uint64_t w0 = *reinterpret_cast<const uint64_t*>(pa);
        const uint64_t w1 = pa + 8 < tend ? *reinterpret_cast<const uint64_t*>(pa + 8) : 0ull;
        const uint64_t w2 = pa + 16 < tend ? *reinterpret_cast<const uint64_t*>(pa + 16) : 0ull;
        const uint64_t b0 = sh ? (w0 >> sh) | (w1 << (64u - sh)) : w0;
        const uint64_t b1 = sh ? (w1 >> sh) | (w2 << (64u - sh)) : w1;
        uint32_t used = 0, cov = 1;
        while ((uint64_t)cov < len && cov < 200u) {
            const uint32_t byte = cov < 8u ? (uint32_t)(b0 >> (8u * cov)) & 0xFFu : (cov < 16u ? (uint32_t)(b1 >> (8u * (cov - 8u))) & 0xFFu : (uint32_t)q[cov]);
            used += vl_len[byte];
            if (used > vl_kb1) break;
            ++cov;
        }
        hcov[j] = (uint8_t)cov;
        h = (uint64_t)cov + h_extra;
    }
    uint64_t key2 = 0;
    if constexpr (USE_ISA) {
        key2 = (uint64_t)rank[ds + d + off + h];
    } else {
        const uint64_t rem = doc_start[d + 1] - ds - off - h;
        const uint8_t* p = text + ds + off + h;
        if (nsym2 <= 9 && rem > 0) {
            const uint64_t pa = (uint64_t)p & ~7ull;
            const uint32_t sh = (uint32_t)((uint64_t)p & 7ull) * 8u;
            const uint64_t w0 = *reinterpret_cast<const uint64_t*>(pa);
            const uint64_t w1 = pa + 8 < (uint64_t)(text + n_text) ? *reinterpret_cast<const uint64_t*>(pa + 8) : 0ull;
            const uint64_t lo = sh ? (w0 >> sh) | (w1 << (64u - sh)) : w0;
            const uint32_t b8 = (uint32_t)(w1 >> sh) & 0xFFu;
            for (int k = 0; k < nsym2; ++k) {
                const uint32_t byte = k < 8 ? (uint32_t)(lo >> (8 * k)) & 0xFFu : b8;
                const uint64_t sym = (uint64_t)k < rem ? (uint64_t)symmap[byte] : 0ull;
                key2 = (key2 << symbits) | sym;
            }
        } else {
            for (int k = 0; k < nsym2; ++k) {
                const uint64_t sym = (uint64_t)k < rem ? (uint64_t)symmap[p[k]] : 0ull;
                key2 = (key2 << symbits) | sym;
            }
        }
    }
    skey[j] |= key2;
}
// ... 89 lines not shown
                }
            }
            cpre += ctot;
        }
        const uint32_t total = cpre & 0xFFFFu;
        __builtin_amdgcn_fence(__ATOMIC_RELEASE, "wavefront");
        __builtin_amdgcn_wave_barrier();
        __builtin_amdgcn_fence(__ATOMIC_ACQUIRE, "wavefront");
        uint32_t heads = 0;
        for (uint32_t b0 = 0; b0 < total; b0 += 64u) {
            const uint32_t t = b0 + (uint32_t)lane;
            const bool live = t < total;
            const uint32_t e = live ? (uint32_t)list[t] : 0u;
            const uint32_t head = (e >> 12) & 1u;
            const uint64_t hb = __builtin_amdgcn_ballot_w64(head != 0);
            if (live) {
                const U2 run{tile_run.a + t, tile_run.b + heads + (uint64_t)__popcll(hb & lt_mask)};
                const U2 nxt{run.a + 1, run.b + head};
                out(tile * SC_TILE + (uint64_t)(e & 0xFFFu), run, nxt);
            }
            heads += (uint32_t)__popcll(hb);
        }
        __builtin_amdgcn_fence(__ATOMIC_RELEASE, "wavefront");
        __builtin_amdgcn_wave_barrier();
    }
}

constexpr uint32_t GS_FREE = 32;
template <typename V>
__global__ __launch_bounds__(256) void sa_group_sort_kernel(const uint64_t* __restrict__ kin, const V* __restrict__ vin, uint64_t m, int kbits, uint32_t cap,
                                                            unsigned long long budget, uint64_t* __restrict__ kout, V* __restrict__ vout,
                                                            unsigned long long* __restrict__ state ) {
    const uint64_t j = (uint64_t)blockIdx.x * 256 + threadIdx.x;
    if (j >= m) return;
    const volatile unsigned long long* vstate = state;
    if (vstate[0]) return;
    const uint64_t k = kin[j];
    const uint64_t g = kbits >= 64 ? 0ull : k >> kbits;
    auto gid = [&](uint64_t x) { return kbits >= 64 ? 0ull : x >> kbits; };
    uint64_t pos = j;
    uint32_t walked = 0;
    bool too = false;
    {
        uint32_t d = 1;
        for (; d <= cap && j >= d; ++d) {
            const uint64_t o = kin[j - d];
            if (gid(o) != g) break;
            pos -= (uint64_t)(o > k);
            if ((d & 127u) == 0 && vstate[0]) return;
        }
        too = d > cap && j >= d && gid(kin[j - d]) == g;
        walked += d - 1;
    }
    if (!too) {
        uint32_t d = 1;
        for (; d <= cap && j + d < m; ++d) {
            const uint64_t o = kin[j + d];
            if (gid(o) != g) break;
            pos += (uint64_t)(o < k);
            if ((d & 127u) == 0 && vstate[0]) return;
        }
        too = d > cap && j + d < m && gid(kin[j + d]) == g;
        walked += d - 1;
    }
    if (walked > GS_FREE && !too) too = atomicAdd(&state[1], (unsigned long long)walked) + walked > budget;
    if (too) {
        atomicExch(&state[0], 1ull);
        return;
    }
    kout[pos] = k;
    vout[pos] = vin[j];
}

template <typename I>
__global__ __launch_bounds__(256) void sa_newhead_kernel(const uint64_t* __restrict__ skey, const I* __restrict__ U,
                                                         const uint8_t* __restrict__ flags, uint64_t m,
                                                         uint8_t* __restrict__ nh) {
    const uint64_t j = (uint64_t)blockIdx.x * 256 + threadIdx.x;
    if (j >= m) return;
    const bool oldhead = flags[U[j]] & 1;
    nh[j] = (uint8_t)(oldhead || j == 0 || skey[j] != skey[j - 1]);
}

template <typename SAW, typename I, bool WANT_POS = true>
__device__ __forceinline__ void sa_place(uint64_t j, uint64_t m, const typename SAW::val* sval, const I* U, const uint8_t* nh,
                                         const uint64_t* doc_start, int bits, uint64_t mask, uint64_t hnew, SAW sa,
                                         uint8_t* flags, uint64_t& ext_pos, unsigned long long* still_open,
                                         const uint8_t* hcov = nullptr, uint32_t h_add = 0, uint8_t* lf = nullptr) {
    if (hcov) hnew = (uint64_t)hcov[j] + h_add;
    const typename SAW::val v = sval[j];
    const uint64_t i = U[j];
    const bool head = nh[j];
    const bool last = j + 1 == m || nh[j + 1];
    const uint64_t d = (uint64_t)v & mask, off = (uint64_t)v >> bits;
    uint64_t ds = 0;
    bool exhausted = false;
    if (WANT_POS || !(head && last)) {
        ds = doc_start[d];
        exhausted = doc_start[d + 1] - ds - off < hnew;
    }
    const bool open = !(head && last) && !exhausted;
    sa.store(i, v);
    flags[i] = (uint8_t)((head ? 1 : 0) | (open ? 2 : 0));
    if (lf) lf[j] = (uint8_t)((head ? 1 : 0) | (open ? 2 : 0));
    if (open) atomicAdd(still_open, 1ull);
    ext_pos = ds + d + off;
}

template <typename SAW, typename I>
__global__ __launch_bounds__(256) void sa_update_kernel(const typename SAW::val* __restrict__ sval, const I* __restrict__ U,
                                                        const uint8_t* __restrict__ nh, uint64_t m,
                                                        const uint64_t* __restrict__ doc_start, int bits,
                                                        uint64_t mask, uint64_t hnew, SAW sa,
                                                        uint8_t* __restrict__ flags,
                                                        unsigned long long* __restrict__ still_open,
                                                        const uint8_t* __restrict__ hcov = nullptr, uint32_t h_add = 0, uint8_t* __restrict__ lf = nullptr) {
    const uint64_t j = (uint64_t)blockIdx.x * 256 + threadIdx.x;
    if (j >= m) return;
    uint64_t q;
    sa_place<SAW, I, false>(j, m, sval, U, nh, doc_start, bits, mask, hnew, sa, flags, q, still_open, hcov, h_add, lf);
}

template <typename I>
struct HeadIn {
    const uint8_t* nh;
    const I* U;
    __device__ __forceinline__ uint64_t operator()(uint64_t j) const { return nh[j] ? (uint64_t)U[j] + 1 : 0ull; }
};
struct SlotOrder {
    const unsigned long long* a_start = nullptr;
    const unsigned long long* u_start = nullptr;
    uint32_t nseg = 0;
    __device__ __forceinline__ uint64_t operator()(uint64_t slot) const {
        if (nseg == 0) return slot;
        uint32_t lo = 0, hi = nseg - 1;
        while (lo < hi) {
            const uint32_t mid = lo + (hi - lo + 1) / 2;
            if (a_start[mid] <= slot) lo = mid; else hi = mid - 1;
        }
        return slot - a_start[lo] + u_start[lo];
    }
};

template <typename SAW, typename I, typename R>
struct UpdateOut {
    using V = typename SAW::val;
    const V* sval;
    const I* U;
    const uint8_t* nh;
    uint64_t m;
    const uint64_t* doc_start;
    int bits;
    uint64_t mask, hnew;
    SAW sa;
    uint8_t* flags;
    R* rank;
    unsigned long long* still_open;
    SlotOrder order;
    __device__ __forceinline__ void operator()(uint64_t j, uint64_t, uint64_t incl) const {
        uint64_t q;
        sa_place<SAW, I>(j, m, sval, U, nh, doc_start, bits, mask, hnew, sa, flags, q, still_open);
        rank[q] = (R)(order(incl - 1) + 1);
    }
};

struct AllHeadIn {
    const uint8_t* flags;
    __device__ __forceinline__ uint64_t operator()(uint64_t i) const { return (flags[i] & 1) ? i + 1 : 0ull; }
};
template <typename SAW, typename R>
struct IsaOut {
    SAW sa;
    const uint64_t* doc_start;
    int bits;
    uint64_t mask;
    R* rank;
    SlotOrder order;
    __device__ __forceinline__ void operator()(uint64_t i, uint64_t, uint64_t incl) const {
        const auto v = sa.load(i);
        const uint64_t d = (uint64_t)v & mask, off = (uint64_t)v >> bits;
        rank[doc_start[d] + d + off] = (R)(order(incl - 1) + 1);
    }
};

struct CompatBucket {
    unsigned long long lo, hi;
};

template <typename V>
__global__ __launch_bounds__(320) void compat_bounds_kernel(typename SaOf<V>::ptr sa,
                                                            const uint8_t* __restrict__ text,
                                                            const uint64_t* __restrict__ doc_start, int bits,
                                                            uint64_t mask, const CompatBucket* __restrict__ buckets,
                                                            uint64_t depth, unsigned long long* __restrict__ bounds) {
    const int c = threadIdx.x;
    if (c > 257) return;
    const CompatBucket b = buckets[blockIdx.x];
    uint64_t lo = b.lo, hi = b.hi;
    if (c == 257) {
        bounds[(uint64_t)blockIdx.x * 258 + c] = b.hi;
        return;
    }
    while (lo < hi) {
// ... 551 lines not shown
        CDB_HIP(hipMemcpyAsync(dh.h_top.data(), tc.totals, 256 * sizeof(uint64_t), hipMemcpyDeviceToHost, s));
        CDB_HIP(hipStreamSynchronize(s));
        st.msd_first = 2;
    } else if (msd_span) {
        dh.msd_m = (unsigned long long)msd_span * kbase * kbase * kbase * kbase;
        const uint32_t tiles8 = (uint32_t)ceil_div(n, (uint64_t)RS_GEN8_TILE);
        tc.d_tc.alloc((size_t)tiles8 * 256 * sizeof(uint32_t));
        int t = ix.prof.begin(s);
        hipLaunchKernelGGL(sa_tile_paircount_kernel, dim3((unsigned)ceil_div((uint64_t)tiles8, (uint64_t)(4 * TPC_TILES_PER_WAVE))), dim3(256), 0, s, text, n,
                           (const uint16_t*)al.d_symmap.as<uint16_t>(), kbase, dh.pair_consts.pair_r, dh.pair_consts.pair_s, tiles8, tc.d_tc.as<uint32_t>());
        hipLaunchKernelGGL(sa_tile_docend_fix_kernel, dim3((unsigned)std::max<uint64_t>(1, std::min<uint64_t>(ceil_div(D, 256), 1024))), dim3(256), 0, s,
                           text, doc_start, D, n, (const uint16_t*)al.d_symmap.as<uint16_t>(), kbase, dh.pair_consts.pair_r, dh.pair_consts.pair_s,
                           tc.d_tc.as<uint32_t>());
        tc.totals = rs_tile_totals(s, ix.tbw, tc.d_tc.as<uint32_t>(), tiles8, nullptr);
        ix.prof.end(t, "sa_tile_paircount", n + D * 18 + (uint64_t)tiles8 * 2048, s);
        dh.h_top.assign(256, 0);
        CDB_HIP(hipMemcpyAsync(dh.h_top.data(), tc.totals, 256 * sizeof(uint64_t), hipMemcpyDeviceToHost, s));
        CDB_HIP(hipStreamSynchronize(s));
        tc.counted = true;
        st.msd_first = 2;
    } else if (fused && dense) {
        const int npass = (int)ceil_div(key_bits, 8);
        key_histograms(npass, use_msd ? 1u << (npass - 1) : 0xFFFFFFFFu);
        if (use_msd) dh.h_top.assign(h_hist.begin() + (size_t)(npass - 1) * 256, h_hist.begin() + (size_t)npass * 256);
    } else if (fused && !big) {
        DevBuf d_corr;
        const size_t corr_words = (size_t)HC_MAXSYM * 257 + HC_MAXSYM;
        d_corr.alloc(corr_words * sizeof(uint64_t));
        CDB_HIP(hipMemsetAsync(d_corr.p, 0, corr_words * sizeof(uint64_t), s));
        {
            const int grid = (int)std::min<uint64_t>(ceil_div(D, 256), 256 * 4);
            int t = ix.prof.begin(s);
            hipLaunchKernelGGL(sa_headcorr_kernel, dim3(std::max(grid, 1)), dim3(256), 0, s, text, doc_start, D,
                               (const uint16_t*)al.d_symmap.as<uint16_t>(), nsym, d_corr.as<unsigned long long>(),
                               d_corr.as<unsigned long long>() + (size_t)HC_MAXSYM * 257);
            ix.prof.end(t, "sa_headcorr", D * (16 + (uint64_t)nsym), s);
        }
        std::vector<uint64_t> h_corr(corr_words);
        CDB_HIP(hipMemcpyAsync(h_corr.data(), d_corr.p, corr_words * sizeof(uint64_t), hipMemcpyDeviceToHost, s));
        CDB_HIP(hipStreamSynchronize(s));
        const uint64_t* first = h_corr.data();
        const uint64_t* lencnt = h_corr.data() + (size_t)HC_MAXSYM * 257;
        uint64_t code_count[257] = {0};
        for (int b = 0; b < 256; ++b)
            if (al.h_map[b]) code_count[al.h_map[b]] = al.h_counts[b];
        h_hist.assign((size_t)nsym * 256, 0);
        for (int p = 0; p < nsym; ++p) {
            const int k = nsym - 1 - p;
            uint64_t* hp = &h_hist[(size_t)p * 256];
            uint64_t shorter = 0, ends = 0;
            for (int L = 0; L < k; ++L) {
                shorter += lencnt[L];
                ends += (uint64_t)L * lencnt[L];
            }
            hp[0] = ends + (uint64_t)k * (D - shorter);
            for (int c = 1; c <= sigma; ++c) {
                uint64_t head = 0;
                for (int j = 0; j < k; ++j) head += first[(size_t)j * 257 + c];
                hp[c] = code_count[c] - head;
            }
        }
    }
    return dh;
}

struct Depth1Fold {
    uint64_t nend = 0, nlow = 0, nhigh = 0;
    bool fold = false, done = false;
};

struct InitialSort {
    DevBuf sa_buf, flags;
    DevBuf sa_hi_buf;
    bool packed_out = false;
    bool flags_by_sort = false;
    bool tile_sums_ready = false;
    DevBuf sorted_keys, sorted_k32, sorted_low;
    int low_bits = 0, low_bytes = 0;
    std::vector<Depth1Fold> depth1;
    std::vector<CompatBucket> folded_roots;
    uint64_t refine_depth0 = 0;
    DevBuf d_vl_bytelen;
    uint32_t vl_kb1 = 0;
};

template <typename V>
InitialSort initial_sort_direct(Index& ix, const Alphabet& al, const KeyPlan& kp, const DigitHist& dh, TopCounts& tc, SortStats& ss) {
    hipStream_t s = ix.stream;
    const uint64_t n = ix.size, D = ix.ndocs;
    BuildStats& st = ix.bstats;
    const uint8_t* text = ix.d_text;
    const uint64_t* doc_start = ix.d_doc_start.as<uint64_t>();
    const int nsym = kp.nsym, dbits = kp.dbits, key_bits = kp.key_bits;
    const uint32_t kbase = kp.kbase;
    const uint64_t kmagic = kp.kmagic;
    const bool fused = dh.fused, use_msd = dh.use_msd;
    const uint32_t msd_span = dh.msd_span;
    InitialSort out;
    TextGen gen{text, doc_start, al.d_symmap.as<uint16_t>(), D, (int)ix.bits, kbase, nsym, 0, ix.text_padded};
    double ta = now_ms();
    out.flags.alloc(n);
    enum { WIDE, NARROW, SPLIT, SPLIT2 } layout = WIDE;
    if (fused && sizeof(V) == 4 && ix.narrow_keys) {
        if (key_bits <= 32) layout = NARROW;
        else if (key_bits - dbits <= 32) layout = SPLIT;
        else if (key_bits - 2 * dbits <= 32) layout = SPLIT2;
    }
    st.key_layout = (int)layout;
    const int low_bits = out.low_bits = layout == SPLIT ? dbits : (layout == SPLIT2 ? 2 * dbits : 0);
    const int low_bytes = out.low_bytes = layout == SPLIT ? 1 : (layout == SPLIT2 ? 2 : 0);
    if (layout != WIDE) {
        if constexpr (sizeof(V) == 4) {
            DevBuf k32[2], vals[2], low[2];
            k32[0].alloc(n * sizeof(uint32_t));
            k32[1].alloc(n * sizeof(uint32_t));
            vals[0].alloc(n * sizeof(V));
            vals[1].alloc(n * sizeof(V));
            if (low_bytes) {
                if (!use_msd) low[0].alloc(n * low_bytes);
                low[1].alloc(n * low_bytes);
            }
            st.alloc_ms += now_ms() - ta;
            if (getenv("CDB_DEBUG_BUFS"))
                std::fprintf(stderr, "[bufs] k32 %p %p vals %p %p low %p %p flags %p\n", k32[0].p, k32[1].p, vals[0].p, vals[1].p, low[0].p,
                             low[1].p, out.flags.p);
            int sel = 0;
            SegFinalKeepArgs keep;
            DevBuf edges;
            const bool want_keep = ix.flags_in_last_pass && dbits == 8 && rs_variant_maybe_big_atomic(ix.sort_variant, n);
            if (want_keep) {
                const uint64_t nbt = ceil_div(n, (uint64_t)SC_TILE);
                ix.scan_partials.ensure(scan_partials_slots(nbt) * sizeof(U2));
                CDB_HIP(hipMemsetAsync(ix.scan_partials.p, 0, nbt * sizeof(U2), s));
                edges.alloc((ceil_div(n, (uint64_t)RS_SEG_TILE) + 256) * 256 * sizeof(SegEdge));
                keep.flags = out.flags.as<uint8_t>();
                keep.edges = edges.as<SegEdge>();
                keep.low_bits = low_bits;
                keep.kbase = kbase;
                keep.kmagic = kmagic;
                keep.tile_sums = ix.scan_partials.as<unsigned long long>();
                keep.sums_tile = SC_TILE;
            }
            if (layout == SPLIT && use_msd && want_keep) {
                if (msd_span) {
                    gen.msd_pair = true;
                    gen.pair_span = dh.pair_consts.pair_span;
                    gen.pair_r = dh.pair_consts.pair_r;
                    gen.pair_s = dh.pair_consts.pair_s;
                } else {
                    gen.msd_shift = 32;
                }
                const bool prebased = tc.counted && msd_span != 0;
                radix_sort_msd(s, ix.rws, ix.msd_ws, ix.prof, k32[0].as<uint32_t>(), k32[1].as<uint32_t>(), vals[0].as<uint32_t>(),
                               vals[1].as<uint32_t>(), low[1].as<uint8_t>(), n, dh.h_top.data(), gen, dh.msd_m, keep, &ss,
                               prebased ? (const uint32_t*)tc.d_tc.as<uint32_t>() : nullptr, prebased ? &ix.tbw : nullptr, ix.sweep_records);
                st.gen_prebased = prebased ? 1 : 0;
                st.sweep_records = prebased && ix.sweep_records && gen.msd_pair ? 1 : 0;
                tc.d_tc.release();
                ix.tbw.base.release();
                sel = 1;
                out.sorted_low = std::move(low[1]);
                out.flags_by_sort = ix.rws.keep_applied;
            } else if (layout == SPLIT) {
                gen.low_bits = low_bits;
                sel = radix_sort_split<V, uint8_t>(s, ix.rws, ix.prof, k32[0].as<uint32_t>(), k32[1].as<uint32_t>(),
                                                   vals[0].as<V>(), vals[1].as<V>(), low[0].as<uint8_t>(), low[1].as<uint8_t>(), n,
// ... 282 lines not shown
    const uint16_t* h_map = al.h_map;
    const uint64_t* h_first = bk.first_by_code.data();
    uint64_t at = 0;
    for (int k = 0; k < sigma; ++k) {
        out.folded_roots.push_back(CompatBucket{(unsigned long long)at, (unsigned long long)(at + h_first[bk.border[k]])});
        at += h_first[bk.border[k]];
    }
    st.root_folded = 1;
    bool lo_class = false;
    for (int b = 0; b < 128; ++b) lo_class |= h_map[b] != 0;
    if (lo_class) st.compat_rotations += 1;
    if (!ix.fold_depth1) return;
    DevBuf d_cls;
    d_cls.alloc((512 + 768) * sizeof(uint64_t));
    CDB_HIP(hipMemsetAsync(d_cls.p, 0, (512 + 768) * sizeof(uint64_t), s));
    int t = ix.prof.begin(s);
    if (!al.pair_hi_counted)
    hipLaunchKernelGGL(sa_pairclass_kernel, dim3((unsigned)std::max<uint64_t>(1, std::min<uint64_t>(ceil_div(n, 256 * 16 * 4), 2048))),
                       dim3(256), 0, s, text, n, d_cls.as<unsigned long long>());
    hipLaunchKernelGGL(sa_docend_class_kernel, dim3((unsigned)std::max<uint64_t>(1, std::min<uint64_t>(ceil_div(D, 256), 1024))),
                       dim3(256), 0, s, text, doc_start, D, n, d_cls.as<unsigned long long>() + 512);
    ix.prof.end(t, "sa_pairclass", n + D * 18, s);
    std::vector<uint64_t> cls(512 + 768);
    CDB_HIP(hipMemcpyAsync(cls.data(), d_cls.p, cls.size() * sizeof(uint64_t), hipMemcpyDeviceToHost, s));
    uint64_t h_pair_hi[256];
    if (al.pair_hi_counted) CDB_HIP(hipMemcpyAsync(h_pair_hi, al.d_pair_hi.p, sizeof(h_pair_hi), hipMemcpyDeviceToHost, s));
    CDB_HIP(hipStreamSynchronize(s));
    if (al.pair_hi_counted) {
        for (int b = 0; b < 256; ++b) {
            cls[2 * b + 1] = h_pair_hi[b];
            cls[2 * b] = al.h_counts[b] - h_pair_hi[b];
        }
        st.pairclass_fused = 1;
    }
    const uint64_t chuck1 = std::max<uint64_t>(4096, n / 256);
    out.depth1.assign((size_t)sigma, Depth1Fold{});
    for (int b = 0; b < 256; ++b) {
        if (!h_map[b]) continue;
        const uint64_t* pr = &cls[2 * b];
        const uint64_t* co = &cls[512 + 3 * b];
        Depth1Fold f;
        f.nend = co[2];
        f.nlow = pr[0] - co[0];
        f.nhigh = pr[1] - co[1];
        f.fold = al.h_counts[b] > chuck1 && f.nlow && f.nhigh && f.nend + f.nlow + f.nhigh == al.h_counts[b];
        int slot = 0;
        while (bk.border[slot] != (int)h_map[b]) ++slot;
        out.depth1[slot] = f;
    }
}

struct BucketRecords {
    uint32_t fbase = 0;
    uint64_t bmagic = 0;
    int bpass = 0, lowb = 0;
    int keyb = 4;
    int auxb = 0;
    int recb = 0;
    uint32_t nb = 0;
    std::vector<uint64_t> bstart;
    uint64_t chunk = 2ull << 20;
    uint32_t nch = 0;
    DevBuf d_bstart, d_bounds;
    DevBuf sweep_doc, d_codeslot;
    const unsigned long long* sweep_base = nullptr;
    double avail = 0;
};

template <typename V, typename W>
void run_segmented(Index& ix, const Alphabet& al, const KeyPlan& kp, const Buckets& bk, RecordForm& rf, const BucketRecords& br,
                   uint64_t seg_cap, const DevBuf& d_slotmap, DevBuf& E, InitialSort& out, SortStats& ss, double ta) {
    if constexpr (sizeof(V) == 8) {
        hipStream_t s = ix.stream;
        const uint64_t n = ix.size, D = ix.ndocs;
        BuildStats& st = ix.bstats;
        const uint8_t* text = ix.d_text;
        const uint64_t* doc_start = ix.d_doc_start.as<uint64_t>();
        const int nsym = kp.nsym;
        const uint32_t nb = br.nb, nch = br.nch, bbase = rf.bbase;
        const std::vector<uint64_t>& bstart = br.bstart;
        const int blow = rf.blow, bpass = br.bpass, lowb = br.lowb, recb = br.recb;
        const bool fuse_rec = rf.fuse_rec, sweep_rec = rf.sweep_rec, sweep_fused = rf.sweep_fused, tile_bytes = al.tile_bytes;
        const bool pack_seg = rf.pack_E;
        std::vector<Depth1Fold>& depth1 = out.depth1;
        struct Group {
            uint32_t b0, b1, tiles, cells;
            uint64_t gstart, elems;
            GatherPlan plan;
        };
        std::vector<Group> groups;
        std::vector<SegInfo> h_segs(nb);
        uint32_t max_tiles = 0, max_gb = 0, max_cells = 0;
        uint64_t max_items = 0;
        for (uint32_t b0 = 0; b0 < nb;) {
            uint32_t b1 = b0 + 1;
            while (b1 < nb && bstart[b1 + 1] - bstart[b0] <= seg_cap) ++b1;
            Group g;
            g.b0 = b0;
            g.b1 = b1;
            g.gstart = bstart[b0];
            g.elems = bstart[b1] - bstart[b0];
            uint32_t tiles = 0;
            for (uint32_t b = b0; b < b1; ++b) {
                h_segs[b] = SegInfo{(unsigned long long)(bstart[b] - g.gstart), (unsigned long long)(bstart[b + 1] - g.gstart), tiles, 0u, 0ull, 0ull};
                if (!depth1.empty() && depth1[b].fold) {
                    h_segs[b].rot_a = depth1[b].nend;
                    h_segs[b].rot_b = depth1[b].nend + depth1[b].nlow;
                    depth1[b].done = true;
                    st.compat_rotations += 1;
                }
                tiles += (uint32_t)ceil_div(bstart[b + 1] - bstart[b], (uint64_t)RS_SEG_TILE);
            }
            g.tiles = tiles;
            const uint32_t gb = b1 - b0;
            g.plan.cell_base[0] = 0;
            for (uint32_t x = 0; x < 8; ++x) g.plan.cell_base[x + 1] = g.plan.cell_base[x] + (x < nch ? (nch - x + 7) / 8 : 0u) * gb;
            g.cells = g.plan.cell_base[8];
            max_tiles = std::max(max_tiles, tiles);
            max_gb = std::max(max_gb, gb);
            max_cells = std::max(max_cells, g.cells);
            max_items = std::max<uint64_t>(max_items, g.elems / BR_ITEM + g.cells + 8);
            groups.push_back(g);
            b0 = b1;
        }
        uint64_t max_elems = 0;
        for (const Group& g : groups) max_elems = std::max(max_elems, g.elems);
        DevBuf kb[2], eb[2], wb[2], edges, d_starts, d_segs, tile_seg, cell_off, lists, d_items2, d_bh2;
        uint32_t *kbp[2], *ebp[2];
        const int dead = bpass & 1;
        for (int q = 0; q < 2; ++q) {
            if (fuse_rec) {
                kb[q] = std::move(rf.fr_kv[q]);
                kbp[q] = kb[q].as<uint32_t>();
                if (out.packed_out) {
                    eb[q] = std::move(rf.fr_e[q]);
                    ebp[q] = eb[q].as<uint32_t>();
                } else {
                    ebp[q] = kbp[q] + max_elems;
                }
                wb[q] = std::move(rf.fr_w[q]);
                continue;
            } else {
                kb[q].alloc(max_elems * sizeof(uint32_t));
                eb[q].alloc(max_elems * sizeof(uint32_t));
                kbp[q] = kb[q].as<uint32_t>();
                ebp[q] = eb[q].as<uint32_t>();
            }
            wb[q].alloc(max_elems * sizeof(W));
        }
        edges.alloc((size_t)max_tiles * 256 * sizeof(SegEdge));
        d_starts.alloc((size_t)max_gb * 8 * 256 * sizeof(uint64_t));
        d_bh2.alloc((size_t)max_gb * 8 * 256 * sizeof(uint64_t));
        d_segs.alloc((size_t)nb * sizeof(SegInfo));
        tile_seg.alloc((size_t)max_tiles * sizeof(uint32_t));
        cell_off.alloc((size_t)max_cells * sizeof(uint32_t));
        lists.alloc(groups.size() * 16 * sizeof(uint32_t));
        d_items2.alloc((size_t)max_items * sizeof(BucketItem));
        st.alloc_ms += now_ms() - ta;
        CDB_HIP(hipMemcpyAsync(d_segs.p, h_segs.data(), (size_t)nb * sizeof(SegInfo), hipMemcpyHostToDevice, s));
        CDB_HIP(hipMemsetAsync(lists.p, 0, groups.size() * 16 * sizeof(uint32_t), s));
        const unsigned long long* bnd = br.d_bounds.as<unsigned long long>();
        for (size_t gi = 0; gi < groups.size(); ++gi) {
            const Group& g = groups[gi];
            const uint32_t gb = g.b1 - g.b0;
            uint32_t* list_len = lists.as<uint32_t>() + gi * 16;
            uint32_t* tickets = list_len + 8;
            if (fuse_rec && !sweep_fused) {
                {
                    hipLaunchKernelGGL(rs_seg_tilemap_kernel, dim3((unsigned)ceil_div(g.tiles, 256)), dim3(256), 0, s,
                                       (const SegInfo*)(d_segs.as<SegInfo>() + g.b0), gb, g.tiles, tile_seg.as<uint32_t>());
                    TextGen rg{text, doc_start, al.d_symmap.as<uint16_t>(), D, (int)ix.bits, bbase, nsym, 0, ix.text_padded};
                    rg.slotmap = d_slotmap.as<uint8_t>();
                    rg.rec_low_bits = blow;
                    radix_gen_records<W>(s, ix.rws, ix.prof, kbp[0], ebp[0], wb[0].as<W>(), n,
                                         bk.first_digit.data(), rg, (const uint32_t*)tile_seg.as<uint32_t>(),
                                         (const SegInfo*)(d_segs.as<SegInfo>() + g.b0), gb, g.tiles, lowb, bpass,
                                         d_bh2.as<unsigned long long>(), &ss,
                                         tile_bytes ? (const uint32_t*)al.d_tbc.as<uint32_t>() : nullptr,
                                         tile_bytes ? (const uint16_t*)bk.d_src_col.as<uint16_t>() : nullptr, tile_bytes ? &ix.tbw : nullptr);
                    st.gen_prebased = tile_bytes ? 1 : 0;
                }
            } else if (sweep_rec || sweep_fused) {
                hipLaunchKernelGGL(rs_seg_tilemap_kernel, dim3((unsigned)ceil_div(g.tiles, 256)), dim3(256), 0, s,
                                   (const SegInfo*)(d_segs.as<SegInfo>() + g.b0), gb, g.tiles, tile_seg.as<uint32_t>());
                TextGen rg{text, doc_start, al.d_symmap.as<uint16_t>(), D, (int)ix.bits, bbase, nsym, 0, ix.text_padded};
                rg.slotmap = d_slotmap.as<uint8_t>();
                rg.rec_low_bits = blow;
                rg.part_m = rf.part_m;
                rg.part_r = rf.part_gen.part_r;
                rg.part_s = rf.part_gen.part_s;
                rg.tile_doc = br.sweep_doc.as<uint64_t>();
                rg.tile_base = br.sweep_base;
                if (rf.vl_bits) {
                    VlTables vt;
                    vt.sym = rf.d_vl_sym.as<uint16_t>();
                    vt.dec = rf.d_vl_dec.as<uint16_t>();
                    vt.key_bits = rf.vl_bits;
                    vt.end_len = rf.vlc.end_len;
                    radix_sweep_records_vl<W>(s, ix.prof, kbp[0], ebp[0], wb[0].as<W>(), n, rg, (const uint16_t*)br.d_codeslot.as<uint16_t>(), vt,
                                              g.b0, g.b1, g.gstart, g.elems, (const uint32_t*)tile_seg.as<uint32_t>(),
                                              (const SegInfo*)(d_segs.as<SegInfo>() + g.b0), gb, g.tiles, lowb, bpass,
                                              d_bh2.as<unsigned long long>(), &ss);
                } else
                radix_sweep_records<W>(s, ix.prof, kbp[0], ebp[0], wb[0].as<W>(), n, rg, (const uint16_t*)br.d_codeslot.as<uint16_t>(), g.b0, g.b1,
                                       g.gstart, g.elems,
                                       (const uint32_t*)tile_seg.as<uint32_t>(), (const SegInfo*)(d_segs.as<SegInfo>() + g.b0), gb,
                                       g.tiles, lowb, bpass, d_bh2.as<unsigned long long>(), &ss);
                st.sweep_records = 1;
                st.gen_prebased = 1;
            } else {
            CDB_HIP(hipMemsetAsync(d_bh2.p, 0, (size_t)gb * 8 * 256 * sizeof(uint64_t), s));
            int t = ix.prof.begin(s);
            hipLaunchKernelGGL(sa_gather_plan_kernel, dim3(8), dim3(1024), 0, s, bnd, nch, g.b0, gb, g.plan, cell_off.as<uint32_t>(),
                               list_len);
            hipLaunchKernelGGL(sa_gather_emit_kernel, dim3((unsigned)ceil_div(g.cells, 256)), dim3(256), 0, s, bnd, nch, g.b0, gb,
                               g.plan, (const uint32_t*)cell_off.as<uint32_t>(), (const uint32_t*)list_len,
                               d_items2.as<BucketItem>());
            ix.prof.end(t, "sa_gather_plan", (uint64_t)g.cells * 24 + (g.elems / BR_ITEM) * sizeof(BucketItem), s);
            t = ix.prof.begin(s);
            constexpr unsigned gather_wgs = 256u * 8u;
            if (pack_seg)
            hipLaunchKernelGGL((sa_bucket_records_lists_kernel<W, Packed40>), dim3(gather_wgs), dim3(256), 0, s,
                               Sa40{E.as<uint32_t>(), out.sa_hi_buf.as<uint8_t>()},
                               (const BucketItem*)d_items2.as<BucketItem>(), (const uint32_t*)list_len, tickets, text, n, doc_start,
                               (const uint16_t*)al.d_symmap.as<uint16_t>(), (int)ix.bits, ix.mask, nsym, bbase, blow, bpass, g.gstart,
                               g.b0, kbp[0], wb[0].as<W>(), ebp[0], d_bh2.as<unsigned long long>());
            else
            hipLaunchKernelGGL((sa_bucket_records_lists_kernel<W>), dim3(gather_wgs), dim3(256), 0, s, (const uint64_t*)E.as<uint64_t>(),
                               (const BucketItem*)d_items2.as<BucketItem>(), (const uint32_t*)list_len, tickets, text, n, doc_start,
                               (const uint16_t*)al.d_symmap.as<uint16_t>(), (int)ix.bits, ix.mask, nsym, bbase, blow, bpass, g.gstart,
                               g.b0, kbp[0], wb[0].as<W>(), ebp[0], d_bh2.as<unsigned long long>());
            ix.prof.end(t, "sa_bucket_records", g.elems * ((uint64_t)nsym + recb + sizeof(V)), s);
            st.gather_items += g.elems / BR_ITEM;
            hipLaunchKernelGGL(rs_seg_tilemap_kernel, dim3((unsigned)ceil_div(g.tiles, 256)), dim3(256), 0, s,
                               (const SegInfo*)(d_segs.as<SegInfo>() + g.b0), gb, g.tiles, tile_seg.as<uint32_t>());
            }
            SegFinalArgs fin;
            if (pack_seg) {
                fin.elo = E.as<uint32_t>() + g.gstart;
                fin.ehi = out.sa_hi_buf.as<uint8_t>() + g.gstart;
            } else if (out.packed_out) {
                fin.elo = kbp[dead] + g.gstart;
                fin.ehi = out.sa_hi_buf.as<uint8_t>() + g.gstart;
            } else {
                fin.eout = (fuse_rec ? kb[dead].as<uint64_t>() : E.as<uint64_t>()) + g.gstart;
            }
            fin.flags = out.flags.as<uint8_t>() + g.gstart;
            fin.edges = edges.as<SegEdge>();
            fin.hi_shift = blow;
            fin.low_bits = blow;
            fin.kbase = br.fbase;
            fin.kmagic = br.bmagic;
            radix_sort_segmented<W>(s, ix.rws, ix.prof, kbp[0], kbp[1], ebp[0], ebp[1], wb[0].as<W>(), wb[1].as<W>(), g.elems,
                                    (const SegInfo*)(d_segs.as<SegInfo>() + g.b0), (const uint32_t*)tile_seg.as<uint32_t>(), gb,
                                    g.tiles, (const unsigned long long*)d_bh2.as<unsigned long long>(),
                                    d_starts.as<unsigned long long>(), rf.bbits - blow, lowb, fin, &ss);
            st.bucket_groups++;
        }
        CDB_HIP(hipStreamSynchronize(s));
        if (sweep_rec || sweep_fused) ix.tbw.base.release();
        if (fuse_rec) E = std::move(kb[dead]);
        if (pack_seg) out.packed_out = true;
        st.segmented = 1;
    }
}

template <typename V, typename I>
void run_per_bucket(Index& ix, const Alphabet& al, const KeyPlan& kp, const Buckets& bk, const RecordForm& rf, const BucketRecords& br,
                    DevBuf& E, InitialSort& out, SortStats& ss) {
    hipStream_t s = ix.stream;
    const uint64_t n = ix.size;
    BuildStats& st = ix.bstats;
    const uint8_t* text = ix.d_text;
    const uint64_t* doc_start = ix.d_doc_start.as<uint64_t>();
    const int nsym = kp.nsym;
    const uint32_t nb = br.nb, nch = br.nch, bbase = rf.bbase;
    const std::vector<uint64_t>& bstart = br.bstart;
    const int bbits = rf.bbits, blow = rf.blow, bpass = br.bpass, lowb = br.lowb, keyb = br.keyb, auxb = br.auxb, recb = br.recb;
    const bool packed = rf.packed;
    const uint64_t maxb = bk.maxb, bmagic = br.bmagic;
    const double avail = br.avail;
    std::vector<uint64_t> bounds((size_t)nb * (nch + 1));
    CDB_HIP(hipMemcpyAsync(bounds.data(), br.d_bounds.p, bounds.size() * 8, hipMemcpyDeviceToHost, s));
    CDB_HIP(hipStreamSynchronize(s));
    const bool third = !packed && avail > (double)maxb * (2.0 * (keyb + lowb) + 2 * sizeof(V)) * 1.15;
    const double scratch = packed ? (double)maxb * recb
                                  : (double)maxb * (keyb + lowb + (third ? 2 : 1) * sizeof(V)) +
                                        (third ? (double)(n / 32) * (sizeof(I) + 16 + 2 * sizeof(V) + 1) : 0.0);
    uint64_t gcap = (uint64_t)std::max(0.0, (avail - scratch) * 0.85 / recb);
    if (ix.bucket_group_limit) gcap = std::min<uint64_t>(gcap, ix.bucket_group_limit);
    gcap = std::max<uint64_t>(std::min<uint64_t>(gcap, n), maxb);
    DevBuf k32g, lowg, k32t, lowt, ET, EX, elog, elot, d_bh, d_items;
    k32g.alloc(gcap * keyb);
    if (auxb) lowg.alloc(gcap * auxb);
    k32t.alloc(maxb * keyb);
    if (auxb) lowt.alloc(maxb * auxb);
    if (packed) {
        elog.alloc(gcap * sizeof(uint32_t));
        elot.alloc(maxb * sizeof(uint32_t));
    } else {
        ET.alloc(maxb * sizeof(V));
        if (third) EX.alloc(maxb * sizeof(V));
    }
    std::vector<uint64_t> bh;
    std::vector<BucketItem> items;
    auto run_group = [&](auto wtag, auto ktag, uint32_t b0, uint32_t b1) {
        using W = decltype(wtag);
        using K = decltype(ktag);
        constexpr bool HAS_W = !std::is_same<W, NoVal>::value;
        using FW = typename std::conditional<HAS_W, W, uint8_t>::type;
        const uint64_t gstart = bstart[b0];
        const uint32_t gb = b1 - b0;
        d_bh.ensure((size_t)gb * 8 * 256 * sizeof(uint64_t));
        CDB_HIP(hipMemsetAsync(d_bh.p, 0, (size_t)gb * 8 * 256 * sizeof(uint64_t), s));
        items.clear();
        for (uint32_t x = 0; x < nch; ++x)
            for (uint32_t b = b0; b < b1; ++b) {
                const uint64_t lo = bounds[(size_t)b * (nch + 1) + x], hi = bounds[(size_t)b * (nch + 1) + x + 1];
                for (uint64_t o = lo; o < hi; o += BR_ITEM)
                    items.push_back(BucketItem{(unsigned long long)o, (uint32_t)std::min<uint64_t>(BR_ITEM, hi - o), b});
            }
        st.gather_items += items.size();
        if (!items.empty()) {
            d_items.ensure(items.size() * sizeof(BucketItem));
            CDB_HIP(hipMemcpyAsync(d_items.p, items.data(), items.size() * sizeof(BucketItem), hipMemcpyHostToDevice, s));
            int t = ix.prof.begin(s);
            hipLaunchKernelGGL((sa_bucket_records_kernel<V, W, K>), dim3((unsigned)items.size()), dim3(256), 0, s,
                               (const V*)E.as<V>(), (const BucketItem*)d_items.as<BucketItem>(), text, n, doc_start,
                               (const uint16_t*)al.d_symmap.as<uint16_t>(), (int)ix.bits, ix.mask, nsym, bbase, blow, bpass,
                               gstart, b0, k32g.as<K>(), lowg.as<W>(), d_bh.as<unsigned long long>());
            ix.prof.end(t, "sa_bucket_records", (bstart[b1] - gstart) * ((uint64_t)nsym + keyb + lowb + sizeof(V)), s);
        }
        CDB_HIP(hipStreamSynchronize(s));
        for (uint32_t b = b0; b < b1; ++b) {
            const uint64_t start = bstart[b], cnt = bstart[b + 1] - start;
// ... 288 lines not shown
        ix.key_nsym = kp.nsym;
        ix.key_base = kp.kbase;
    } else {
        is.sorted_keys.release();
        is.sorted_k32.release();
        is.sorted_low.release();
    }
    ix.bstats.free_ms += now_ms() - ta;
}

struct RefineBuffers {
    DevBuf d_order;
    DevBuf U, skey[2], sval[2], nh, rank, hcov;
    DevBuf d_open;
    DevBuf U2b, lf;
    DevBuf d_gs_state;
};

SlotOrder make_slot_order(Index& ix, const InitialSort& is, const Alphabet& al, DevBuf& d_order) {
    SlotOrder order;
    if (is.folded_roots.empty()) return order;
    const std::vector<Depth1Fold>& depth1 = is.depth1;
    struct Blk { unsigned long long a, len; int code, cls; };
    std::vector<Blk> blks;
    std::vector<int> code_of_root;
    {
        for (int b = 128; b < 256; ++b) if (al.h_map[b]) code_of_root.push_back(al.h_map[b]);
        for (int b = 0; b < 128; ++b) if (al.h_map[b]) code_of_root.push_back(al.h_map[b]);
    }
    for (size_t b = 0; b < is.folded_roots.size(); ++b) {
        const CompatBucket r = is.folded_roots[b];
        if (!depth1.empty() && depth1[b].done) {
            blks.push_back(Blk{r.lo, depth1[b].nend, code_of_root[b], 0});
            blks.push_back(Blk{r.lo + depth1[b].nend, depth1[b].nhigh, code_of_root[b], 2});
            blks.push_back(Blk{r.lo + depth1[b].nend + depth1[b].nhigh, depth1[b].nlow, code_of_root[b], 1});
        } else {
            blks.push_back(Blk{r.lo, r.hi - r.lo, code_of_root[b], 0});
        }
    }
    std::vector<size_t> by_u(blks.size());
    for (size_t i = 0; i < by_u.size(); ++i) by_u[i] = i;
    std::sort(by_u.begin(), by_u.end(), [&](size_t x, size_t y) {
        return blks[x].code != blks[y].code ? blks[x].code < blks[y].code : blks[x].cls < blks[y].cls;
    });
    std::vector<unsigned long long> tab(2 * blks.size());
    unsigned long long at = 0;
    for (size_t i : by_u) {
        tab[blks.size() + i] = at;
        at += blks[i].len;
    }
    for (size_t i = 0; i < blks.size(); ++i) tab[i] = blks[i].a;
    d_order.alloc(tab.size() * sizeof(unsigned long long));
    CDB_HIP(hipMemcpyAsync(d_order.p, tab.data(), tab.size() * sizeof(unsigned long long), hipMemcpyHostToDevice, ix.stream));
    CDB_HIP(hipStreamSynchronize(ix.stream));
    order.a_start = d_order.as<unsigned long long>();
    order.u_start = d_order.as<unsigned long long>() + blks.size();
    order.nseg = (uint32_t)blks.size();
    return order;
}

template <typename V, typename I, typename R, typename SAW>
uint64_t refine_groups(Index& ix, SAW sa, InitialSort& is, const Alphabet& al, const KeyPlan& kp, SortStats& ss, RefineBuffers& rb) {
    hipStream_t s = ix.stream;
    const uint64_t n = ix.size, D = ix.ndocs;
    BuildStats& st = ix.bstats;
    const uint8_t* text = ix.d_text;
    const uint64_t* doc_start = ix.d_doc_start.as<uint64_t>();
    const int symbits = al.symbits;
    const DevBuf& flags = is.flags;
    const uint32_t vl_kb1 = is.vl_kb1;
    const SlotOrder order = make_slot_order(ix, is, al, rb.d_order);
    DevBuf &U = rb.U, (&skey)[2] = rb.skey, (&sval)[2] = rb.sval, &nh = rb.nh, &rank = rb.rank, &hcov = rb.hcov;
    DevBuf &d_open = rb.d_open, &U2b = rb.U2b, &lf = rb.lf, &d_gs_state = rb.d_gs_state;
    uint32_t h_acc = 0;
    uint64_t h = is.refine_depth0 ? is.refine_depth0 : (uint64_t)kp.nsym;
    bool isa = false;
    uint64_t cap = 0;
    d_open.alloc(sizeof(uint64_t));
    bool have_list = false;
    uint64_t m_list = 0;
    int list_rs = 0;
    d_gs_state.alloc(2 * sizeof(unsigned long long));
    bool group_sort_on = ix.group_sort;
    for (;;) {
        if (st.rounds > 0) {
            uint64_t still = 0;
            CDB_HIP(hipMemcpyAsync(&still, d_open.p, sizeof(still), hipMemcpyDeviceToHost, s));
            CDB_HIP(hipStreamSynchronize(s));
            if (still == 0) break;
        }
        CDB_HIP(hipMemsetAsync(d_open.p, 0, sizeof(uint64_t), s));
        auto flag_tile_sums = [&]() {
            const uint64_t nb = ceil_div(n, SC_TILE);
            ix.scan_partials.ensure(scan_partials_slots(nb) * sizeof(U2));
            int t = ix.prof.begin(s);
            hipLaunchKernelGGL(sa_flag_count_kernel, dim3((unsigned)ceil_div(nb, (uint64_t)(4 * FC_TILES_PER_WAVE))), dim3(256), 0, s,
                               (const uint8_t*)flags.as<uint8_t>(), n, nb, ix.scan_partials.as<U2>());
            ix.prof.end(t, "sa_flag_count", n, s);
        };
        bool from_list = have_list && ix.list_rounds;
        have_list = false;
        if (from_list) {
            const uint64_t nb = ceil_div(m_list, SC_TILE);
            ix.scan_partials.ensure(scan_partials_slots(nb) * sizeof(U2));
            int t = ix.prof.begin(s);
            hipLaunchKernelGGL(sa_flag_count_kernel, dim3((unsigned)ceil_div(nb, (uint64_t)(4 * FC_TILES_PER_WAVE))), dim3(256), 0, s,
                               (const uint8_t*)lf.as<uint8_t>(), m_list, nb, ix.scan_partials.as<U2>());
            ix.prof.end(t, "sa_flag_count", m_list, s);
        } else if (!is.tile_sums_ready) {
            flag_tile_sums();
        }
        U2 tot = scan_totals_from_partials<U2>(s, ix.scan_partials, from_list ? m_list : n, OpAdd{}, U2{0, 0});
        is.tile_sums_ready = false;
        uint64_t m = tot.a, G = tot.b;
        if (st.rounds == 0) st.unresolved_initial = m;
        st.unresolved_max = std::max(st.unresolved_max, m);
        if (m == 0) break;
        if (m >= (1ull << 32) - 4096) throw InternalError("too many unresolved suffixes for one refinement round (internal limit: 2^32)");
        const int gbits = bit_width64(G - 1);
        int nsym2 = std::min((64 - gbits) / symbits, KG_LOOK);
        if (!isa) {
            const bool use_text = !ix.force_doubling && nsym2 >= 1 &&
                                  ((m <= n / 32 && st.ext_rounds < 4) || (m <= n / 8 && st.ext_rounds < 2));
            if (!use_text) {
                rank.alloc((n + D + 1) * sizeof(R));
                CDB_HIP(hipMemsetAsync(rank.p, 0, (n + D + 1) * sizeof(R), s));
                AllHeadIn ain{flags.as<uint8_t>()};
                (void)scan_totals<uint64_t>(s, ix.scan_partials, ain, n, OpMax{}, (uint64_t)0);
                IsaOut<SAW, R> iout{sa, doc_start, (int)ix.bits, ix.mask, rank.as<R>(), order};
                int t = ix.prof.begin(s);
                scan_apply<uint64_t>(s, ix.scan_partials, ain, n, OpMax{}, (uint64_t)0, iout);
                ix.prof.end(t, "sa_isa_init", n * (1 + sizeof(V) + sizeof(R)), s);
                isa = true;
                st.isa_built = 1;
                from_list = false;
                flag_tile_sums();
                (void)scan_totals_from_partials<U2>(s, ix.scan_partials, n, OpAdd{}, U2{0, 0});
            }
        }
        const int kbits = isa ? bit_width64(n) : nsym2 * symbits;
        if (kbits + gbits > 64) throw InternalError("refinement key does not fit 64 bits (internal limit)");
        if (m > cap) {
            cap = m;
            U.alloc(m * sizeof(I));
            skey[0].alloc(m * 8);
            skey[1].alloc(m * 8);
            sval[0].alloc(m * sizeof(V));
            sval[1].alloc(m * sizeof(V));
            nh.alloc(m);
            lf.alloc(m + 16);
            if (vl_kb1) hcov.alloc(m);
        }
        {
            int t = ix.prof.begin(s);
            if (from_list) {
                if (list_rs == 0) {
                    std::swap(skey[0], skey[1]);
                    std::swap(sval[0], sval[1]);
                    list_rs = 1;
                }
                U2b.ensure(cap * sizeof(I));
                CompactListOut<V, I> co{(const I*)U.as<I>(), (const V*)sval[1].as<V>(), U2b.as<I>(), skey[0].as<uint64_t>(), sval[0].as<V>(), kbits};
                hipLaunchKernelGGL((sa_flag_compact_kernel<decltype(co)>), dim3((unsigned)ceil_div(ceil_div(m_list, SC_TILE), (uint64_t)(4 * FC_TILES_PER_WAVE))),
                                   dim3(256), 0, s, (const uint8_t*)lf.as<uint8_t>(), m_list, (uint64_t)ceil_div(m_list, SC_TILE),
                                   (const U2*)ix.scan_partials.as<U2>(), co);
                std::swap(U, U2b);
                st.list_rounds++;
            } else {
            CompactOut<SAW, I> co{sa, U.as<I>(), skey[0].as<uint64_t>(), sval[0].as<V>(), kbits};
            hipLaunchKernelGGL((sa_flag_compact_kernel<decltype(co)>), dim3((unsigned)ceil_div(ceil_div(n, SC_TILE), (uint64_t)(4 * FC_TILES_PER_WAVE))),
                               dim3(256), 0, s, (const uint8_t*)flags.as<uint8_t>(), n, (uint64_t)ceil_div(n, SC_TILE),
                               (const U2*)ix.scan_partials.as<U2>(), co);
            }
            if (isa)
                hipLaunchKernelGGL((sa_round_keys_kernel<V, R, true>), dim3((unsigned)ceil_div(m, 256)), dim3(256), 0, s,
                                   (const V*)sval[0].as<V>(), m, doc_start, text, (const uint16_t*)al.d_symmap.as<uint16_t>(),
                                   (const R*)rank.as<R>(), (int)ix.bits, ix.mask, h, nsym2, symbits, skey[0].as<uint64_t>(), n);
            else
                hipLaunchKernelGGL((sa_round_keys_kernel<V, R, false>), dim3((unsigned)ceil_div(m, 256)), dim3(256), 0, s,
                                   (const V*)sval[0].as<V>(), m, doc_start, text, (const uint16_t*)al.d_symmap.as<uint16_t>(),
                                   (const R*)nullptr, (int)ix.bits, ix.mask, h, nsym2, symbits, skey[0].as<uint64_t>(), n,
                                   vl_kb1 ? (const uint8_t*)is.d_vl_bytelen.as<uint8_t>() : nullptr, vl_kb1, h_acc, vl_kb1 ? hcov.as<uint8_t>() : nullptr);
            ix.prof.end(t, "sa_compact", n + m * (sizeof(I) + 8 + 2 * sizeof(V)), s);
        }
        int rs = -1;
        if (group_sort_on) {
            CDB_HIP(hipMemsetAsync(d_gs_state.p, 0, 2 * sizeof(unsigned long long), s));
            int t = ix.prof.begin(s);
            hipLaunchKernelGGL((sa_group_sort_kernel<V>), dim3((unsigned)ceil_div(m, 256)), dim3(256), 0, s, (const uint64_t*)skey[0].as<uint64_t>(),
                               (const V*)sval[0].as<V>(), m, kbits, (uint32_t)ix.group_sort_cap, (unsigned long long)(16 * m + (1u << 20)),
                               skey[1].as<uint64_t>(), sval[1].as<V>(), d_gs_state.as<unsigned long long>());
            ix.prof.end(t, "sa_group_sort", m * 2 * (8 + sizeof(V)), s);
            unsigned long long gave_up = 0;
            CDB_HIP(hipMemcpyAsync(&gave_up, d_gs_state.p, sizeof(gave_up), hipMemcpyDeviceToHost, s));
            CDB_HIP(hipStreamSynchronize(s));
            if (gave_up) {
                group_sort_on = false;
                st.group_sort_fallbacks++;
            } else {
                rs = 1;
                st.group_sorts++;
            }
        }
        if (rs < 0) {
            rs = radix_sort<uint64_t, V>(s, ix.rws, ix.prof, skey[0].as<uint64_t>(), skey[1].as<uint64_t>(),
                                         sval[0].as<V>(), sval[1].as<V>(), m, 0, kbits + gbits, &ss, ix.sort_variant);
            radix_check_error(s, ix.rws);
        }
        hipLaunchKernelGGL((sa_newhead_kernel<I>), dim3((unsigned)ceil_div(m, 256)), dim3(256), 0, s,
                           (const uint64_t*)skey[rs].as<uint64_t>(), (const I*)U.as<I>(),
                           (const uint8_t*)flags.as<uint8_t>(), m, nh.as<uint8_t>());
        const uint64_t hnew = isa ? 2 * h : h + (uint64_t)nsym2;
        {
            int t = ix.prof.begin(s);
            if (isa) {
                HeadIn<I> hin{nh.as<uint8_t>(), U.as<I>()};
                (void)scan_totals<uint64_t>(s, ix.scan_partials, hin, m, OpMax{}, (uint64_t)0);
                UpdateOut<SAW, I, R> uo{sval[rs].as<V>(), U.as<I>(), nh.as<uint8_t>(), m, doc_start, (int)ix.bits,
                                      ix.mask, hnew, sa, flags.as<uint8_t>(), rank.as<R>(), d_open.as<unsigned long long>(), order};
                scan_apply<uint64_t>(s, ix.scan_partials, hin, m, OpMax{}, (uint64_t)0, uo);
                st.dbl_rounds++;
            } else {
                hipLaunchKernelGGL((sa_update_kernel<SAW, I>), dim3((unsigned)ceil_div(m, 256)), dim3(256), 0, s,
                                   (const V*)sval[rs].as<V>(), (const I*)U.as<I>(), (const uint8_t*)nh.as<uint8_t>(), m,
                                   doc_start, (int)ix.bits, ix.mask, hnew, sa, flags.as<uint8_t>(), d_open.as<unsigned long long>(),
                                   vl_kb1 ? (const uint8_t*)hcov.as<uint8_t>() : nullptr, h_acc + (uint32_t)nsym2, lf.as<uint8_t>());
                h_acc += (uint32_t)nsym2;
                st.ext_rounds++;
                have_list = true;
                m_list = m;
                list_rs = rs;
            }
            ix.prof.end(t, "sa_update", m * (2 * sizeof(V) + sizeof(I) + 2 + (isa ? sizeof(R) : 0)), s);
        }
        h = hnew;
        st.rounds++;
        if (st.rounds > 80) throw InternalError("suffix-array refinement did not converge (internal error)");
    }
    return h;
}

template <typename V>
void finish_reference_order(Index& ix, InitialSort& is, Alphabet& al) {
    ix.sa_sorted = !(ix.reference_compat && al.high_bytes);
    ix.pivot_levels = 0;
    if (ix.key_nsym) {
        ix.d_symmap_q = std::move(al.d_symmap);
        std::memcpy(ix.h_symmap_q, al.h_map, sizeof(al.h_map));
    }
    if (ix.reference_compat && al.high_bytes) {
        std::vector<CompatBucket>& folded_roots = is.folded_roots;
        const std::vector<Depth1Fold>& depth1 = is.depth1;
        if (!folded_roots.empty() && !depth1.empty()) {
            std::vector<CompatBucket> nodes;
            for (size_t b = 0; b < folded_roots.size(); ++b) {
                const CompatBucket r = folded_roots[b];
                if (depth1[b].done) {
                    const unsigned long long hs = r.lo + depth1[b].nend, ls = hs + depth1[b].nhigh;
                    if (depth1[b].nend) nodes.push_back(CompatBucket{r.lo, hs});
                    nodes.push_back(CompatBucket{hs, ls});
                    nodes.push_back(CompatBucket{ls, r.hi});
                } else {
                    nodes.push_back(r);
                }
            }
            folded_roots.swap(nodes);
        }
        const std::vector<CompatBucket>* roots = folded_roots.empty() ? nullptr : &folded_roots;
        auto reorder = [&](auto tag) {
            using T = decltype(tag);
            if (!apply_reference_order_oop<T>(ix, is.sa_buf, &is.sa_hi_buf, roots)) {
                apply_reference_order<T>(ix, is.sa_buf, &is.sa_hi_buf, roots);
                ix.drop_keys();
            }
        };
        if (is.packed_out) reorder(Packed40{});
        else reorder(V{});
    }
    ix.d_sa = std::move(is.sa_buf);
    ix.d_sa_hi = std::move(is.sa_hi_buf);
    ix.sa_packed = is.packed_out;
}

template <typename V, typename I, typename R>
void build_typed(Index& ix, bool big) {
    hipStream_t s = ix.stream;
    const uint64_t n = ix.size, D = ix.ndocs;
    BuildStats& st = ix.bstats;
    st = BuildStats{};
    {
        const double tf = now_ms();
        ix.release_sa();
        ix.drop_keys();
        ix.d_pivots.release();
        ix.pivot_levels = 0;
        st.free_ms += now_ms() - tf;
    }
    if (n == 0) {
        ix.d_sa.alloc(16);
        ix.sa_sorted = true;
        ix.pivot_levels = 0;
        ix.drop_keys();
        return;
    }
    if (sizeof(R) == 4 && n + D + 2 >= (1ull << 32)) throw InternalError("internal: 32-bit ranks selected for a corpus >= 2^32");
    Alphabet al;
    count_alphabet<V>(ix, big, al);
    TopCounts tc;
    count_top_digits_aside<V>(ix, big, al, tc);
    const KeyPlan kp = plan_keys<V>(ix, big, al);
    const DigitHist dh = digit_histograms<V>(ix, big, al, kp, tc);
    SortStats ss;
    InitialSort is = big ? initial_sort_bucketwise<V, I>(ix, al, kp, ss) : initial_sort_direct<V>(ix, al, kp, dh, tc, ss);
    radix_check_error(s, ix.rws);
    hand_over_keys(ix, big, is, kp);
    RefineBuffers rb;
    uint64_t h;
// ... 133 lines not shown
```

Baseline: 29.74.

## Carry extra variable-length key bits through initial sort to resolve ties cheaply

During the VL-key sweep, up to six extra key bits beyond the sorted prefix are extracted and stashed in spare high bits of the packed entry word, then written into the final flags byte. A new carried refinement round sorts unresolved groups by these carried bits alone, using compaction, a small sort and an update with no text access, before the regular text-extension rounds. This aims to shrink the unresolved set before the more expensive rounds that read text, at the cost of an extra round of compaction, sort and update plus added masking in the hot sweep and final kernels.

```diff
diff --git a/coffeedb_amd/csrc/capi.hip b/coffeedb_amd/csrc/capi.hip
--- a/coffeedb_amd/csrc/capi.hip
+++ b/coffeedb_amd/csrc/capi.hip
@@ -1607,6 +1607,7 @@
     else if (!std::strcmp(name, "partial_symbol")) ix.partial_symbol = value != 0;
     else if (!std::strcmp(name, "group_sort")) ix.group_sort = value != 0;
     else if (!std::strcmp(name, "list_rounds")) ix.list_rounds = value != 0;
+    else if (!std::strcmp(name, "carried_bits")) ix.carried_bits = value < 0 ? -1 : (value > 6 ? 6 : (int)value);
     else if (!std::strcmp(name, "fuse_pairclass")) ix.fuse_pairclass = value != 0;
     else if (!std::strcmp(name, "group_sort_cap")) ix.group_sort_cap = (int)std::max<int64_t>(1, std::min<int64_t>(value, 1 << 20));
     else if (!std::strcmp(name, "vl_keys")) ix.vl_keys = value < 0 ? 0 : (value > 56 ? 56 : (int)value);
@@ -1666,7 +1667,7 @@
         {"build_ms", b.build_ms}, {"alloc_ms", b.alloc_ms}, {"free_ms", b.free_ms}, {"rounds", (double)b.rounds}, {"ext_rounds", (double)b.ext_rounds},
         {"dbl_rounds", (double)b.dbl_rounds}, {"unresolved_after_initial", (double)b.unresolved_initial},
         {"unresolved_max", (double)b.unresolved_max}, {"sort_passes", (double)b.sort_passes},
-        {"sort_passes_skipped", (double)b.sort_passes_skipped}, {"isa_built", (double)b.isa_built}, {"fused_keygen", (double)b.fused_keygen}, {"dense_keys", (double)b.dense_keys}, {"key_layout", (double)b.key_layout}, {"bucketed", (double)b.bucketed}, {"bucket_groups", (double)b.bucket_groups}, {"segmented", (double)b.segmented}, {"fused_records", (double)b.fused_records}, {"sweep_records", (double)b.sweep_records}, {"vl_key_bits", (double)b.vl_key_bits}, {"partial_levels", (double)b.partial_levels}, {"list_rounds", (double)b.list_rounds}, {"pairclass_fused", (double)b.pairclass_fused}, {"group_sorts", (double)b.group_sorts}, {"group_sort_fallbacks", (double)b.group_sort_fallbacks}, {"vl_avg_len", b.vl_avg_len}, {"vl_rate", b.vl_rate}, {"vl_est_unresolved", b.vl_est_unresolved}, {"fixed_est_unresolved", b.fixed_est_unresolved}, {"gen_prebased", (double)b.gen_prebased}, {"root_folded", (double)b.root_folded}, {"flags_in_last_pass", (double)b.flags_in_last_pass}, {"msd_first", (double)b.msd_first}, {"bucket_low_digits", (double)b.bucket_low_digits}, {"key_directory_cells", h->ix.h_keydir.empty() ? 0.0 : (double)(h->ix.h_keydir.size() - 1)}, {"group_fallbacks", (double)h->ix.group_fallbacks}, {"dense_key_retries", (double)h->ix.dense_key_retries}, {"self_check_fallbacks", (double)h->ix.self_check_fallbacks}, {"sa_packed", h->ix.sa_packed ? 1.0 : 0.0}, {"sa_bytes_per_entry", h->ix.sa_packed ? 5.0 : (double)h->ix.width}, {"self_check_pairs", (double)h->ix.self_check_pairs}, {"self_check_ms", h->ix.self_check_ms}, {"self_check_coverage", h->ix.size > 1 ? (double)h->ix.self_check_pairs / (double)(h->ix.size - 1) : 0.0},
+        {"sort_passes_skipped", (double)b.sort_passes_skipped}, {"isa_built", (double)b.isa_built}, {"fused_keygen", (double)b.fused_keygen}, {"dense_keys", (double)b.dense_keys}, {"key_layout", (double)b.key_layout}, {"bucketed", (double)b.bucketed}, {"bucket_groups", (double)b.bucket_groups}, {"segmented", (double)b.segmented}, {"fused_records", (double)b.fused_records}, {"sweep_records", (double)b.sweep_records}, {"vl_key_bits", (double)b.vl_key_bits}, {"partial_levels", (double)b.partial_levels}, {"list_rounds", (double)b.list_rounds}, {"pairclass_fused", (double)b.pairclass_fused}, {"group_sorts", (double)b.group_sorts}, {"group_sort_fallbacks", (double)b.group_sort_fallbacks}, {"carried_key_bits", (double)b.carried_key_bits}, {"carried_rounds", (double)b.carried_rounds}, {"unresolved_after_carried", (double)b.unresolved_after_carried}, {"vl_avg_len", b.vl_avg_len}, {"vl_rate", b.vl_rate}, {"vl_est_unresolved", b.vl_est_unresolved}, {"fixed_est_unresolved", b.fixed_est_unresolved}, {"gen_prebased", (double)b.gen_prebased}, {"root_folded", (double)b.root_folded}, {"flags_in_last_pass", (double)b.flags_in_last_pass}, {"msd_first", (double)b.msd_first}, {"bucket_low_digits", (double)b.bucket_low_digits}, {"key_directory_cells", h->ix.h_keydir.empty() ? 0.0 : (double)(h->ix.h_keydir.size() - 1)}, {"group_fallbacks", (double)h->ix.group_fallbacks}, {"dense_key_retries", (double)h->ix.dense_key_retries}, {"self_check_fallbacks", (double)h->ix.self_check_fallbacks}, {"sa_packed", h->ix.sa_packed ? 1.0 : 0.0}, {"sa_bytes_per_entry", h->ix.sa_packed ? 5.0 : (double)h->ix.width}, {"self_check_pairs", (double)h->ix.self_check_pairs}, {"self_check_ms", h->ix.self_check_ms}, {"self_check_coverage", h->ix.size > 1 ? (double)h->ix.self_check_pairs / (double)(h->ix.size - 1) : 0.0},
         {"order_proved", (h->ix.proof.state.load() == 2 || h->ix.proof.state.load() == 3 || (h->ix.self_check == 2 && h->ix.width != 0)) ? 1.0 : 0.0},
         {"proof_state", (double)h->ix.proof.state.load()}, {"proof_ms", h->ix.proof.ms}, {"proof_repair_ms", h->ix.proof.repair_ms},
         {"proof_pairs", (double)h->ix.proof.pairs}, {"proof_bad_pairs", (double)h->ix.proof.found[0]}, {"proof_invalid_entries", (double)h->ix.proof.found[1]}, {"proof_skipped_pairs", (double)h->ix.proof.skipped}, {"proof_mixed_pairs", (double)h->ix.proof.mixed},
diff --git a/coffeedb_amd/csrc/index_impl.h b/coffeedb_amd/csrc/index_impl.h
--- a/coffeedb_amd/csrc/index_impl.h
+++ b/coffeedb_amd/csrc/index_impl.h
@@ -40,6 +40,9 @@
     int pairclass_fused = 0;
     int list_rounds = 0;
     int group_sorts = 0, group_sort_fallbacks = 0;
+    int carried_key_bits = 0;
+    int carried_rounds = 0;
+    uint64_t unresolved_after_carried = 0;
     int partial_levels = 0;
     int vl_key_bits = 0;
     double vl_avg_len = 0, vl_rate = 0, vl_est_unresolved = 0, fixed_est_unresolved = 0;
@@ -260,6 +263,7 @@
     bool segmented_sort = true;
     bool fuse_records = true;
     bool fuse_pairclass = true;
+    int carried_bits = -1;
     bool list_rounds = true;
     int group_sort_cap = 4096;
     bool group_sort = true;
diff --git a/coffeedb_amd/csrc/radix_sort.h b/coffeedb_amd/csrc/radix_sort.h
--- a/coffeedb_amd/csrc/radix_sort.h
+++ b/coffeedb_amd/csrc/radix_sort.h
@@ -214,6 +214,9 @@
     int low_bits = 0;
     uint32_t kbase = 2;
     unsigned long long kmagic = 0;
+    uint32_t hi_mask = 0xFFFFFFFFu;
+    uint32_t carry_mask = 0;
+    int carry_shift = 0;
 };
 
 struct SegFinalKeepArgs : SegArgs {
@@ -991,6 +994,7 @@
                         if (!exhausted) f |= 2u;
                     }
                     if constexpr (FINAL) {
+                        f |= (((uint32_t)s_aux[HAS_W ? i : 0] >> seg.carry_shift) & seg.carry_mask) << 2;
                         if (!(RS_SEG_ABL & 1)) seg.flags[rs_seg_rotated(si, s_gbase[dd] + i)] = (uint8_t)f;
                         continue;
                     } else {
@@ -1035,7 +1039,7 @@
             if constexpr (FINAL) {
                 if (i < valid && !(RS_SEG_ABL & 2)) {
                     const unsigned long long slot = rs_seg_rotated(si, s_gbase[dig[j]] + i);
-                    const uint32_t hi32 = (uint32_t)s_aux[HAS_W ? i : 0] >> seg.hi_shift;
+                    const uint32_t hi32 = ((uint32_t)s_aux[HAS_W ? i : 0] >> seg.hi_shift) & seg.hi_mask;
                     if (seg.elo) {
                         seg.elo[slot] = (uint32_t)s_vals[i];
                         seg.ehi[slot] = (uint8_t)hi32;
diff --git a/coffeedb_amd/csrc/records_sweep.h b/coffeedb_amd/csrc/records_sweep.h
--- a/coffeedb_amd/csrc/records_sweep.h
+++ b/coffeedb_amd/csrc/records_sweep.h
@@ -1,5 +1,6 @@
 #pragma once
 #include "radix_sort.h"
+#include "vl_code.h"
 
 namespace cdb {
 
@@ -290,6 +291,8 @@
     const uint16_t* dec = nullptr;
     int key_bits = 0;
     int end_len = 0;
+    int carry = 0;
+    int carry_shift = 0;
 };
 constexpr uint32_t RS_VL_BITW = ((RS_GEN8_TILE + RS_GEN_LOOK) * 7 + 31) / 32 + 4;
 
@@ -516,7 +519,8 @@
     __syncthreads();
 
     const int KB1 = vl.key_bits - 1;
-    const uint64_t lmask = (1ull << gen.rec_low_bits) - 1ull;
+    const int CX = vl.carry, KBX = KB1 + CX;
+    const uint64_t lmask = (1ull << gen.rec_low_bits) - 1ull, cmask = (1ull << CX) - 1ull;
     auto emit = [&](uint32_t p, uint32_t li, uint64_t e64, uint32_t endbit) {
         const uint32_t o0 = s_boff[li];
         const uint32_t wi = o0 >> 5, sh = o0 & 31u;
@@ -526,14 +530,15 @@
         const uint32_t dv = s_dec[(uint32_t)(top >> 57)];
         const uint32_t sl = dv & 0xFFu, len = dv >> 8;
         const uint32_t avail = endbit - (o0 + len);
-        const uint32_t take = avail < (uint32_t)KB1 ? avail : (uint32_t)KB1;
-        uint64_t kb = (top << len) >> (64 - KB1);
-        kb &= ~0ull << ((uint32_t)KB1 - take);
+        const uint32_t take = avail < (uint32_t)KBX ? avail : (uint32_t)KBX;
+        uint64_t kbx = (top << len) >> (64 - KBX);
+        kbx &= ~0ull << ((uint32_t)KBX - take);
+        const uint64_t kb = kbx >> CX;
         const uint64_t key = (kb << 1) | (uint64_t)(avail + (uint32_t)vl.end_len > (uint32_t)KB1 ? 1u : 0u);
         const uint64_t dst = s_gbase[sl] + (uint64_t)p;
         kout[dst] = (uint32_t)(key >> gen.rec_low_bits);
         vout[dst] = (uint32_t)e64;
-        wout[dst] = (W)((key & lmask) | ((e64 >> 32) << gen.rec_low_bits));
+        wout[dst] = (W)((key & lmask) | ((e64 >> 32) << gen.rec_low_bits) | ((kbx & cmask) << vl.carry_shift));
     };
     if (docs_in_lds && s_flag == 0 && valid == (uint32_t)TILE) {
         const int bits = gen.bits;
@@ -855,6 +860,8 @@
                             SortStats* stats) {
     if (!gen_in.tile_base || !gen_in.tile_doc || !d_codeslot || !vl.sym || !vl.dec) throw InternalError("radix_sweep_records_vl: tables missing (internal)");
     if (vl.key_bits < 16 || vl.key_bits > 56) throw InternalError("radix_sweep_records_vl: key width (internal)");
+    if (vl.carry < 0 || VL_MAX_LEN + vl.key_bits - 1 + vl.carry > 64 || (vl.carry && vl.carry_shift + vl.carry > 8 * (int)sizeof(W)))
+        throw InternalError("radix_sweep_records_vl: carried bits (internal)");
     const uint32_t tiles8 = (uint32_t)ceil_div(n, (uint64_t)RS_SWEEP_TILE);
     const uint32_t grid = (uint32_t)(ceil_div(tiles8, 8u * RS_GROUP) * 8u * RS_GROUP);
     CDB_HIP(hipMemsetAsync(d_hist_out, 0, (size_t)nseg * 8 * 256 * sizeof(uint64_t), s));
diff --git a/coffeedb_amd/csrc/sa_build.hip b/coffeedb_amd/csrc/sa_build.hip
--- a/coffeedb_amd/csrc/sa_build.hip
+++ b/coffeedb_amd/csrc/sa_build.hip
@@ -1014,6 +1014,24 @@
         const uint64_t j = ex.a;
         U[j] = (I)i;
         skey[j] = (in.b - 1) << kbits;
+        sval[j] = sa.load(i);
+    }
+};
+
+template <typename SAW, typename I>
+struct CompactCarriedOut {
+    using V = typename SAW::val;
+    SAW sa;
+    const uint8_t* flags;
+    I* U;
+    uint64_t* skey;
+    V* sval;
+    int kbits;
+    __device__ __forceinline__ void operator()(uint64_t i, const U2& ex, const U2& in) const {
+        if (in.a == ex.a) return;
+        const uint64_t j = ex.a;
+        U[j] = (I)i;
+        skey[j] = ((in.b - 1) << kbits) | (uint64_t)(((uint32_t)flags[i] >> 2) & ((1u << kbits) - 1u));
         sval[j] = sa.load(i);
     }
 };
@@ -1269,7 +1287,7 @@
     nh[j] = (uint8_t)(oldhead || j == 0 || skey[j] != skey[j - 1]);
 }
 
-template <typename SAW, typename I, bool WANT_POS = true>
+template <typename SAW, typename I, bool WANT_POS = true, bool CARRIED = false>
 __device__ __forceinline__ void sa_place(uint64_t j, uint64_t m, const typename SAW::val* sval, const I* U, const uint8_t* nh,
                                          const uint64_t* doc_start, int bits, uint64_t mask, uint64_t hnew, SAW sa,
                                          uint8_t* flags, uint64_t& ext_pos, unsigned long long* still_open,
@@ -1282,7 +1300,7 @@
     const uint64_t d = (uint64_t)v & mask, off = (uint64_t)v >> bits;
     uint64_t ds = 0;
     bool exhausted = false;
-    if (WANT_POS || !(head && last)) {
+    if (!CARRIED && (WANT_POS || !(head && last))) {
         ds = doc_start[d];
         exhausted = doc_start[d + 1] - ds - off < hnew;
     }
@@ -1290,11 +1308,11 @@
     sa.store(i, v);
     flags[i] = (uint8_t)((head ? 1 : 0) | (open ? 2 : 0));
     if (lf) lf[j] = (uint8_t)((head ? 1 : 0) | (open ? 2 : 0));
-    if (open) atomicAdd(still_open, 1ull);
+    if (!CARRIED && open) atomicAdd(still_open, 1ull);
     ext_pos = ds + d + off;
 }
 
-template <typename SAW, typename I>
+template <typename SAW, typename I, bool CARRIED = false>
 __global__ __launch_bounds__(256) void sa_update_kernel(const typename SAW::val* __restrict__ sval, const I* __restrict__ U,
                                                         const uint8_t* __restrict__ nh, uint64_t m,
                                                         const uint64_t* __restrict__ doc_start, int bits,
@@ -1305,7 +1323,7 @@
     const uint64_t j = (uint64_t)blockIdx.x * 256 + threadIdx.x;
     if (j >= m) return;
     uint64_t q;
-    sa_place<SAW, I, false>(j, m, sval, U, nh, doc_start, bits, mask, hnew, sa, flags, q, still_open, hcov, h_add, lf);
+    sa_place<SAW, I, false, CARRIED>(j, m, sval, U, nh, doc_start, bits, mask, hnew, sa, flags, q, still_open, hcov, h_add, lf);
 }
 
 template <typename I>
@@ -2023,6 +2041,7 @@
     uint64_t refine_depth0 = 0;
     DevBuf d_vl_bytelen;
     uint32_t vl_kb1 = 0;
+    uint32_t carry = 0;
 };
 
 template <typename V>
@@ -2471,6 +2490,15 @@
         const int blow = rf.blow, bpass = br.bpass, lowb = br.lowb, recb = br.recb;
         const bool fuse_rec = rf.fuse_rec, sweep_rec = rf.sweep_rec, sweep_fused = rf.sweep_fused, tile_bytes = al.tile_bytes;
         const bool pack_seg = rf.pack_E;
+        const int ehb = std::max(0, (int)ix.bits + ix.off_bits - 32);
+        int carry = 0;
+        if (rf.vl_bits && (sweep_rec || sweep_fused)) {
+            carry = std::min({8 - ehb, 6, 64 - VL_MAX_LEN - (rf.vl_bits - 1)});
+            if (ix.carried_bits >= 0) carry = std::min(carry, ix.carried_bits);
+            carry = std::max(carry, 0);
+        }
+        out.carry = (uint32_t)carry;
+        st.carried_key_bits = carry;
         std::vector<Depth1Fold>& depth1 = out.depth1;
         struct Group {
             uint32_t b0, b1, tiles, cells;
@@ -2586,6 +2614,8 @@
                     vt.dec = rf.d_vl_dec.as<uint16_t>();
                     vt.key_bits = rf.vl_bits;
                     vt.end_len = rf.vlc.end_len;
+                    vt.carry = carry;
+                    vt.carry_shift = blow + ehb;
                     radix_sweep_records_vl<W>(s, ix.prof, kbp[0], ebp[0], wb[0].as<W>(), n, rg, (const uint16_t*)br.d_codeslot.as<uint16_t>(), vt,
                                               g.b0, g.b1, g.gstart, g.elems, (const uint32_t*)tile_seg.as<uint32_t>(),
                                               (const SegInfo*)(d_segs.as<SegInfo>() + g.b0), gb, g.tiles, lowb, bpass,
@@ -2640,6 +2670,11 @@
             fin.low_bits = blow;
             fin.kbase = br.fbase;
             fin.kmagic = br.bmagic;
+            if (carry) {
+                fin.hi_mask = (1u << ehb) - 1u;
+                fin.carry_mask = (1u << carry) - 1u;
+                fin.carry_shift = blow + ehb;
+            }
             radix_sort_segmented<W>(s, ix.rws, ix.prof, kbp[0], kbp[1], ebp[0], ebp[1], wb[0].as<W>(), wb[1].as<W>(), g.elems,
                                     (const SegInfo*)(d_segs.as<SegInfo>() + g.b0), (const uint32_t*)tile_seg.as<uint32_t>(), gb,
                                     g.tiles, (const unsigned long long*)d_bh2.as<unsigned long long>(),
@@ -3094,13 +3129,19 @@
     int list_rs = 0;
     d_gs_state.alloc(2 * sizeof(unsigned long long));
     bool group_sort_on = ix.group_sort;
-    for (;;) {
-        if (st.rounds > 0) {
+    const uint32_t carry = is.carry;
+    bool carried_pending = carry > 0, list_is_carried = false;
+    uint32_t kb_shared = vl_kb1;
+    st.carried_rounds = 0;
+    for (uint32_t iter = 0;; ++iter) {
+        if (iter > 0 && !list_is_carried) {
             uint64_t still = 0;
             CDB_HIP(hipMemcpyAsync(&still, d_open.p, sizeof(still), hipMemcpyDeviceToHost, s));
             CDB_HIP(hipStreamSynchronize(s));
             if (still == 0) break;
         }
+        const bool carried = carried_pending;
+        carried_pending = false;
         CDB_HIP(hipMemsetAsync(d_open.p, 0, sizeof(uint64_t), s));
         auto flag_tile_sums = [&]() {
             const uint64_t nb = ceil_div(n, SC_TILE);
@@ -3125,13 +3166,14 @@
         U2 tot = scan_totals_from_partials<U2>(s, ix.scan_partials, from_list ? m_list : n, OpAdd{}, U2{0, 0});
         is.tile_sums_ready = false;
         uint64_t m = tot.a, G = tot.b;
-        if (st.rounds == 0) st.unresolved_initial = m;
+        if (iter == 0) st.unresolved_initial = st.unresolved_after_carried = m;
+        if (list_is_carried) st.unresolved_after_carried = m;
         st.unresolved_max = std::max(st.unresolved_max, m);
         if (m == 0) break;
         if (m >= (1ull << 32) - 4096) throw InternalError("too many unresolved suffixes for one refinement round (internal limit: 2^32)");
         const int gbits = bit_width64(G - 1);
         int nsym2 = std::min((64 - gbits) / symbits, KG_LOOK);
-        if (!isa) {
+        if (!isa && !carried) {
             const bool use_text = !ix.force_doubling && nsym2 >= 1 &&
                                   ((m <= n / 32 && st.ext_rounds < 4) || (m <= n / 8 && st.ext_rounds < 2));
             if (!use_text) {
@@ -3150,7 +3192,7 @@
                 (void)scan_totals_from_partials<U2>(s, ix.scan_partials, n, OpAdd{}, U2{0, 0});
             }
         }
-        const int kbits = isa ? bit_width64(n) : nsym2 * symbits;
+        const int kbits = carried ? (int)carry : (isa ? bit_width64(n) : nsym2 * symbits);
         if (kbits + gbits > 64) throw InternalError("refinement key does not fit 64 bits (internal limit)");
         if (m > cap) {
             cap = m;
@@ -3177,14 +3219,20 @@
                                    dim3(256), 0, s, (const uint8_t*)lf.as<uint8_t>(), m_list, (uint64_t)ceil_div(m_list, SC_TILE),
                                    (const U2*)ix.scan_partials.as<U2>(), co);
                 std::swap(U, U2b);
-                st.list_rounds++;
+                if (!list_is_carried) st.list_rounds++;
+            } else if (carried) {
+                CompactCarriedOut<SAW, I> co{sa, (const uint8_t*)flags.as<uint8_t>(), U.as<I>(), skey[0].as<uint64_t>(), sval[0].as<V>(), kbits};
+                hipLaunchKernelGGL((sa_flag_compact_kernel<decltype(co)>), dim3((unsigned)ceil_div(ceil_div(n, SC_TILE), (uint64_t)(4 * FC_TILES_PER_WAVE))),
+                                   dim3(256), 0, s, (const uint8_t*)flags.as<uint8_t>(), n, (uint64_t)ceil_div(n, SC_TILE),
+                                   (const U2*)ix.scan_partials.as<U2>(), co);
             } else {
             CompactOut<SAW, I> co{sa, U.as<I>(), skey[0].as<uint64_t>(), sval[0].as<V>(), kbits};
             hipLaunchKernelGGL((sa_flag_compact_kernel<decltype(co)>), dim3((unsigned)ceil_div(ceil_div(n, SC_TILE), (uint64_t)(4 * FC_TILES_PER_WAVE))),
                                dim3(256), 0, s, (const uint8_t*)flags.as<uint8_t>(), n, (uint64_t)ceil_div(n, SC_TILE),
                                (const U2*)ix.scan_partials.as<U2>(), co);
             }
-            if (isa)
+            if (carried) {
+            } else if (isa)
                 hipLaunchKernelGGL((sa_round_keys_kernel<V, R, true>), dim3((unsigned)ceil_div(m, 256)), dim3(256), 0, s,
                                    (const V*)sval[0].as<V>(), m, doc_start, text, (const uint16_t*)al.d_symmap.as<uint16_t>(),
                                    (const R*)rank.as<R>(), (int)ix.bits, ix.mask, h, nsym2, symbits, skey[0].as<uint64_t>(), n);
@@ -3192,7 +3240,7 @@
                 hipLaunchKernelGGL((sa_round_keys_kernel<V, R, false>), dim3((unsigned)ceil_div(m, 256)), dim3(256), 0, s,
                                    (const V*)sval[0].as<V>(), m, doc_start, text, (const uint16_t*)al.d_symmap.as<uint16_t>(),
                                    (const R*)nullptr, (int)ix.bits, ix.mask, h, nsym2, symbits, skey[0].as<uint64_t>(), n,
-                                   vl_kb1 ? (const uint8_t*)is.d_vl_bytelen.as<uint8_t>() : nullptr, vl_kb1, h_acc, vl_kb1 ? hcov.as<uint8_t>() : nullptr);
+                                   vl_kb1 ? (const uint8_t*)is.d_vl_bytelen.as<uint8_t>() : nullptr, kb_shared, h_acc, vl_kb1 ? hcov.as<uint8_t>() : nullptr);
             ix.prof.end(t, "sa_compact", n + m * (sizeof(I) + 8 + 2 * sizeof(V)), s);
         }
         int rs = -1;
@@ -3211,7 +3259,7 @@
                 st.group_sort_fallbacks++;
             } else {
                 rs = 1;
-                st.group_sorts++;
+                if (!carried) st.group_sorts++;
             }
         }
         if (rs < 0) {
@@ -3225,7 +3273,17 @@
         const uint64_t hnew = isa ? 2 * h : h + (uint64_t)nsym2;
         {
             int t = ix.prof.begin(s);
-            if (isa) {
+            if (carried) {
+                hipLaunchKernelGGL((sa_update_kernel<SAW, I, true>), dim3((unsigned)ceil_div(m, 256)), dim3(256), 0, s,
+                                   (const V*)sval[rs].as<V>(), (const I*)U.as<I>(), (const uint8_t*)nh.as<uint8_t>(), m,
+                                   doc_start, (int)ix.bits, ix.mask, (uint64_t)0, sa, flags.as<uint8_t>(), (unsigned long long*)nullptr,
+                                   (const uint8_t*)nullptr, 0u, lf.as<uint8_t>());
+                st.carried_rounds++;
+                kb_shared = vl_kb1 + carry;
+                have_list = true;
+                m_list = m;
+                list_rs = rs;
+            } else if (isa) {
                 HeadIn<I> hin{nh.as<uint8_t>(), U.as<I>()};
                 (void)scan_totals<uint64_t>(s, ix.scan_partials, hin, m, OpMax{}, (uint64_t)0);
                 UpdateOut<SAW, I, R> uo{sval[rs].as<V>(), U.as<I>(), nh.as<uint8_t>(), m, doc_start, (int)ix.bits,
@@ -3245,6 +3303,8 @@
             }
             ix.prof.end(t, "sa_update", m * (2 * sizeof(V) + sizeof(I) + 2 + (isa ? sizeof(R) : 0)), s);
         }
+        list_is_carried = carried;
+        if (carried) continue;
         h = hnew;
         st.rounds++;
         if (st.rounds > 80) throw InternalError("suffix-array refinement did not converge (internal error)");
```

After: 30.89, median of 6. 1.04x the previous value.
